# CostaLab/PILOT

Measured on AMD Instinct MI355X. Metric: W2 patient-pairs/sec (full NxN EMD matrix), higher is better.
Workload: dtype f32 (products as 2-way fp16 splits, 22 significant bits, on the f16 MFMA, f32 accumulate)

## Files before the change

### pilot_amd/csrc/generic_kernels.hpp

```cpp
#pragma once
#include <hip/hip_runtime.h>

#include "plan_args.hpp"

namespace pilot {

struct GenericParams {
    const double *P, *M;
    int N, K;
    int n_pairs, row_begin, row_step;
    double reg, tau, stop_thr;
    int max_iter, period;
    double *emd; int *iters; double *err; int *flags;
    double *kws;
    int *queue;
    const int *list;
    const int *list_len;
    int nsplit;
};

#ifndef PILOT_GENERIC_WG
#define PILOT_GENERIC_WG 1024
#endif
constexpr int GENERIC_WG = PILOT_GENERIC_WG, GENERIC_WAVES = GENERIC_WG / 64;

__device__ inline double block_reduce_sum(double x, double *red) {
    for (int off = 32; off >= 1; off >>= 1) x += __shfl_xor(x, off);
    const int wave = threadIdx.x / 64, lane = threadIdx.x % 64;
    __syncthreads();
    if (lane == 0) red[wave] = x;
    __syncthreads();
    double s = 0.0;
    for (int w = 0; w < GENERIC_WG / 64; ++w) s += red[w];
    return s;
}
__device__ inline double wave_tree_sum(double x) {
    for (int off = 32; off >= 1; off >>= 1) x += __shfl_xor(x, off);
    return x;
}
__device__ inline double block_reduce_max(double x, double *red) {
    for (int off = 32; off >= 1; off >>= 1) { const double y = __shfl_xor(x, off); x = y > x ? y : x; }
    const int wave = threadIdx.x / 64, lane = threadIdx.x % 64;
    __syncthreads();
    if (lane == 0) red[wave] = x;
    __syncthreads();
    double s = red[0];
    for (int w = 1; w < GENERIC_WG / 64; ++w) s = red[w] > s ? red[w] : s;
    return s;
}

#ifndef PILOT_PLAN_TU
static __global__ void __launch_bounds__(GENERIC_WG) sinkhorn_generic_kernel(GenericParams p) {
    constexpr bool PLAN = false;
    const PlanArgs *pa = nullptr;
#else
static __global__ void __launch_bounds__(GENERIC_WG) sinkhorn_generic_plan_kernel(GenericParams p, PlanArgs plan_args) {
    constexpr bool PLAN = true;
    const PlanArgs *pa = &plan_args;
#endif
    extern __shared__ double sm[];
    const int K = p.K, N = p.N;
    double *a = sm, *b = a + K, *u = b + K, *v = u + K, *up = v + K, *vp = up + K, *alpha = vp + K, *beta = alpha + K;
    double *red = beta + K;
    double *part = red + GENERIC_WAVES;
    int *qs = reinterpret_cast<int *>(part + p.nsplit * K);
    double *Km = p.kws + (size_t)blockIdx.x * 2 * K * K, *Kt = Km + (size_t)K * K;
    const double reg = p.reg;
    auto build_kernel = [&]() {
        for (int t = threadIdx.x; t < K * K; t += GENERIC_WG) {
            const int i = t / K, j = t % K;
            const double val = exp(-(p.M[t] - alpha[i] - beta[j]) / reg);
            Km[t] = val;
            Kt[(size_t)j * K + i] = val;
        }
        __threadfence_block();
        __syncthreads();
    };
    for (;;) {
        if (threadIdx.x == 0) qs[0] = atomicAdd(p.queue, 1);
        __syncthreads();
        const int item = qs[0];
        __syncthreads();
        if (item >= (PLAN ? pa->n_pairs : (p.list_len ? *p.list_len : p.n_pairs))) break;
        const int q = PLAN ? item : p.list ? p.list[item] : item;
        const int i_s = PLAN ? pa->pair_i[item] : p.row_begin + (q / N) * p.row_step, j_s = PLAN ? pa->pair_j[item] : q % N;
        for (int k = threadIdx.x; k < K; k += GENERIC_WG) {
            a[k] = p.P[(size_t)i_s * K + k]; b[k] = p.P[(size_t)j_s * K + k];
            alpha[k] = 0.0; beta[k] = 0.0; u[k] = 1.0 / K; v[k] = 1.0 / K;
        }
        __syncthreads();
        build_kernel();
        double err = 1.0;
        int iters = 0, nabs = 0, last_abs = -1, flags = 0;
        for (int ii = 0; ii < p.max_iter; ++ii) {
            for (int k = threadIdx.x; k < K; k += GENERIC_WG) { up[k] = u[k]; vp[k] = v[k]; }
            __syncthreads();
            const int wave = threadIdx.x / 64, lane = threadIdx.x % 64;
            const int ns = p.nsplit, sw = wave % ns, og = wave / ns, n_og = GENERIC_WAVES / ns;
            const int c0 = (K * sw) / ns, c1 = (K * (sw + 1)) / ns;
            auto product = [&](const double *X, const double *x, const double *num, double *out) {
                for (int j0 = lane + 256 * og; j0 < K; j0 += 256 * n_og) {
                    double s0 = 0.0, s1 = 0.0, s2 = 0.0, s3 = 0.0;
                    const bool h1 = j0 + 64 < K, h2 = j0 + 128 < K, h3 = j0 + 192 < K;
#pragma unroll 8
                    for (int i = c0; i < c1; ++i) {
                        const double xi = x[i];
                        const double *row = X + (size_t)i * K + j0;
                        s0 += row[0] * xi;
                        if (h1) s1 += row[64] * xi;
                        if (h2) s2 += row[128] * xi;
                        if (h3) s3 += row[192] * xi;
                    }
                    part[sw * K + j0] = s0;
                    if (h1) part[sw * K + j0 + 64] = s1;
                    if (h2) part[sw * K + j0 + 128] = s2;
                    if (h3) part[sw * K + j0 + 192] = s3;
                }
                __syncthreads();
                for (int j = threadIdx.x; j < K; j += GENERIC_WG) {
                    double t = part[j];
                    for (int w = 1; w < ns; ++w) t += part[w * K + j];
                    out[j] = num[j] / t;
                }
                __syncthreads();
            };
            product(Km, u, b, v);
            product(Kt, v, a, u);
            iters = ii + 1;
            double mu = 0.0, mv = 0.0, nanf = 0.0;
            for (int k = threadIdx.x; k < K; k += GENERIC_WG) {
                if (u[k] != u[k] || v[k] != v[k]) nanf = 1.0;
                mu = fabs(u[k]) > mu ? fabs(u[k]) : mu;
                mv = fabs(v[k]) > mv ? fabs(v[k]) : mv;
            }
            const bool has_nan = block_reduce_max(nanf, red) > 0.0;
            mu = block_reduce_max(mu, red);
            mv = block_reduce_max(mv, red);
            if (!has_nan && (mu > p.tau || mv > p.tau)) {
                for (int k = threadIdx.x; k < K; k += GENERIC_WG) {
                    alpha[k] += reg * log(u[k]); u[k] = 1.0 / K;
                    beta[k] += reg * log(v[k]); v[k] = 1.0 / K;
                }
                __syncthreads();
                build_kernel();
                ++nabs; last_abs = ii;
            }
            if (ii % p.period == 0) {
                double e2 = 0.0;
                for (int j = wave; j < K; j += GENERIC_WG / 64) {
                    const double lv = log(v[j]);
                    double s = 0.0;
                    for (int i = lane; i < K; i += 64) s += exp(-(p.M[(size_t)i * K + j] - alpha[i] - beta[j]) / reg + log(u[i]) + lv);
                    s = wave_tree_sum(s);
                    if (lane == 0) e2 += (s - b[j]) * (s - b[j]);
                }
                err = sqrt(block_reduce_sum(e2, red));
            }
            if (err <= p.stop_thr) { flags |= 1; break; }
            if (has_nan) {
                for (int k = threadIdx.x; k < K; k += GENERIC_WG) { u[k] = up[k]; v[k] = vp[k]; }
                __syncthreads();
                flags |= 2;
                break;
            }
        }
        if (last_abs >= 0 && last_abs == iters - 1) flags |= 4;
        if (nabs > 0) flags |= 8;
        double val = 0.0;
        for (int t = threadIdx.x; t < K * K; t += GENERIC_WG) {
            const int i = t / K, j = t % K;
            if constexpr (PLAN) {
                const double g = exp(-(p.M[t] - alpha[i] - beta[j]) / reg + log(u[i]) + log(v[j]));
                pa->plans[(size_t)q * K * K + t] = g;
                val += p.M[t] * g;
            } else {
                val += p.M[t] * exp(-(p.M[t] - alpha[i] - beta[j]) / reg + log(u[i]) + log(v[j]));
            }
        }
        val = block_reduce_sum(val, red);
        if (threadIdx.x == 0) {
            p.emd[q] = val;
            if (p.iters) p.iters[q] = iters;
            if (p.err) p.err[q] = err;
            p.flags[q] = flags | 16;
        }
        __syncthreads();
    }
}

}
```

### pilot_amd/csrc/pilot_ot.hip

```cpp
#include <hip/hip_runtime.h>
#include <pthread.h>

#include <chrono>
#include <cmath>
#include <condition_variable>
#include <cstdarg>
#include <cstdio>
#include <cstdlib>
#include <cstring>
#include <map>
#include <mutex>
#include <string>
#include <thread>
#include <new>
#include <vector>

#include "abi_common.hpp"
#include "sinkhorn_launch.hpp"
#include "emd_kernels.hpp"
#include "emd_multi_kernels.hpp"
#include "prepass_kernels.hpp"
#include "cellw2_kernels.hpp"
#include "generic_kernels.hpp"
#include "emd_generic_kernel.hpp"
// ... 130 lines not shown
            bool neg = false;
            for (int d = 0; d < D; ++d) { neg = neg || u[d] < 0.0 || v[d] < 0.0; su += u[d]; sv += v[d]; }
            if (neg || su == 0.0 || sv == 0.0) { out = HUGE_VAL; break; }
            const double ru = 1.0 / su, rv = 1.0 / sv;
            double js = 0.0;
            for (int d = 0; d < D; ++d) {
                const double p = u[d] * ru, q = v[d] * rv, m = (p + q) / 2.0;
                if (p > 0.0) js += p * log(p / m);
                if (q > 0.0) js += q * log(q / m);
            }
            out = sqrt(js / 2.0);
            break;
        }
        case PILOT_OT_METRIC_MAHALANOBIS: {
            double s = 0.0;
            for (int a = 0; a < D; ++a) {
                double t = 0.0;
                for (int b = 0; b < D; ++b) t += (u[b] - v[b]) * aux[(size_t)b * D + a];
                s += t * (u[a] - v[a]);
            }
            out = sqrt(s);
            break;
        }
        default: {
            double s = 0.0;
            for (int d = 0; d < D; ++d) { const double t = fabs(u[d] - v[d]); s = t > s ? t : s; }
            out = s;
        }
        }
        C[(size_t)i * K + j] = out;
        C[(size_t)j * K + i] = out;
    }
}

constexpr int MAX_K = 128;
constexpr int GENERIC_MAX_K = 2048;
constexpr int EMD_MAX_K = 256;
constexpr int WIDE_MAX_K = 256;
constexpr int CTRL_INTS = pilot::CTRL_INTS;
constexpr int CTRL_SHARDS_AT = (CTRL_INTS + 2 * pilot::ORDER_NB + 31) / 32 * 32;
constexpr int CTRL_SHARDS_TRACK_AT = CTRL_SHARDS_AT + pilot::QUEUE_SHARDS * pilot::QUEUE_SHARD_STRIDE;
constexpr int CTRL_BLOCK_INTS = CTRL_SHARDS_TRACK_AT + pilot::QUEUE_SHARDS * pilot::QUEUE_SHARD_STRIDE;
constexpr int TIMING_RING = 64;

constexpr size_t LDS_BYTES = 160 * 1024;
static int emd_nk(int K) { return K <= 64 ? 1 : (K <= 128 ? 2 : (K <= 192 ? 3 : 4)); }
constexpr int EMD_MULTI_MAX_K = 16;
static int emd_multi_mode(int K) {
    const char *e = pilot::test_switch("PILOT_OT_EMD_MULTI");
    if (e && *e) return atoi(e);
    return K <= 15 ? 1 : 2;
}
static int emd_wgs_per_cu(int K) {
    if (K > 128) return 1;
    const size_t lds = pilot::emd_lds_bytes(K);
    int by_lds = (int)(LDS_BYTES / lds);
    const int by_regs = K <= 64 ? 4 : 2;
    if (by_lds > by_regs) by_lds = by_regs;
    return by_lds < 1 ? 1 : by_lds;
}

}

struct pilot_ot_plan {
    int N, K, device;
    double max_cost;
    void *img;
    void *p_slot;
    int *track_list;
    int *track_count;
    int *order_list;
    unsigned char *order_bucket;
    int *order_hist;
    int *flags_ws;
    size_t flags_ws_n;
    int *emd_counter;
    double *f_slab;
    size_t f_slab_bytes;
    double *emdg_slab;
    int emdg_wgs;
    double *kws;
    int generic_wgs;
    float *wide_rec;
    size_t wide_rec_n;
    int *nan_list;
    size_t nan_list_n;
    int n_cu;
    int timing;
    long n_timed;
    long n_calls;
    hipEvent_t ev[TIMING_RING][4];
    int graph_mode;
    int gkey_seen;
    struct GraphKey {
        const void *P, *M, *emd, *iters, *err, *flags;
        double reg, stop_thr, tau, floor_ulps, max_cost;
        int num_iter_max, check_period, cfg, mixed, sym, row_begin, n_rows, row_step, debug;
        bool operator==(const GraphKey &o) const {
            return P == o.P && M == o.M && emd == o.emd && iters == o.iters && err == o.err && flags == o.flags && reg == o.reg &&
                   stop_thr == o.stop_thr && tau == o.tau && floor_ulps == o.floor_ulps && max_cost == o.max_cost && num_iter_max == o.num_iter_max &&
                   check_period == o.check_period && cfg == o.cfg && mixed == o.mixed && sym == o.sym && row_begin == o.row_begin &&
                   n_rows == o.n_rows && row_step == o.row_step && debug == o.debug;
        }
    } gkey;
    hipStream_t gstream;
    hipGraphExec_t gexec;
};

namespace {
std::mutex g_switch_mutex;
std::map<std::string, std::string> g_switches;
}
namespace pilot {
const char *test_switch(const char *name) {
    static thread_local std::string value;
    std::lock_guard<std::mutex> l(g_switch_mutex);
    if (g_switches.empty()) return nullptr;
    auto it = g_switches.find(name);
    if (it == g_switches.end()) return nullptr;
    value = it->second;
    return value.c_str();
}
}

PILOT_API int pilot_ot_test_switch(const char *name, const char *value) {
    std::lock_guard<std::mutex> l(g_switch_mutex);
    if (!name) { g_switches.clear(); return PILOT_OT_OK; }
    if (value) g_switches[name] = value; else g_switches.erase(name);
    return PILOT_OT_OK;
}

PILOT_API int pilot_ot_version(void) { return PILOT_OT_VERSION; }
PILOT_API const char *pilot_ot_last_error(void) { return g_err; }

PILOT_API int pilot_ot_device_count(int *count) {
    if (!count) return fail(PILOT_OT_EINVAL, "count is NULL");
    int n = 0;
    hipError_t e = hipGetDeviceCount(&n);
    if (e != hipSuccess) { (void)hipGetLastError(); n = 0; }
    *count = n;
    return PILOT_OT_OK;
}

PILOT_API int pilot_ot_get_device(int *device) {
    if (!device) return fail(PILOT_OT_EINVAL, "device is NULL");
    HIP_TRY(hipGetDevice(device));
    return PILOT_OT_OK;
}

PILOT_API int pilot_ot_set_device(int device) {
    HIP_TRY(hipSetDevice(device));
    return PILOT_OT_OK;
}

PILOT_API int pilot_ot_device_name(char *buf, int buflen) {
    if (!buf || buflen <= 0) return fail(PILOT_OT_EINVAL, "bad buffer");
    int dev = 0;
    HIP_TRY(hipGetDevice(&dev));
    hipDeviceProp_t prop;
    HIP_TRY(hipGetDeviceProperties(&prop, dev));
    snprintf(buf, buflen, "%s", prop.gcnArchName);
    return PILOT_OT_OK;
}

PILOT_API int pilot_ot_dev_alloc(void **dptr, unsigned long long bytes) {
    if (!dptr) return fail(PILOT_OT_EINVAL, "dptr is NULL");
    HIP_TRY(hipMalloc(dptr, bytes ? bytes : 1));
    return PILOT_OT_OK;
}
PILOT_API int pilot_ot_dev_free(void *dptr) {
    HIP_TRY(hipFree(dptr));
    return PILOT_OT_OK;
}
PILOT_API int pilot_ot_memcpy_h2d(void *dst, const void *src, unsigned long long bytes) {
    HIP_TRY(hipMemcpy(dst, src, bytes, hipMemcpyHostToDevice));
    return PILOT_OT_OK;
}
PILOT_API int pilot_ot_memcpy_d2h(void *dst, const void *src, unsigned long long bytes) {
    HIP_TRY(hipMemcpy(dst, src, bytes, hipMemcpyDeviceToHost));
    return PILOT_OT_OK;
}
PILOT_API int pilot_ot_stream_sync(void *stream) {
    HIP_TRY(hipStreamSynchronize(static_cast<hipStream_t>(stream)));
    return PILOT_OT_OK;
}

namespace { hipError_t ws_get(int slot, size_t bytes, void **out); }

PILOT_API int pilot_ot_cost_matrix_dev_ex(const double *d_centroids, int K, int D, int metric, const double *d_aux, double *d_cost,
                                          void *stream) {
    if (!d_centroids || !d_cost) return fail(PILOT_OT_EINVAL, "NULL pointer");
    if (K <= 0 || D <= 0) return fail(PILOT_OT_EINVAL, "K=%d D=%d must be positive", K, D);
    if (metric < PILOT_OT_METRIC_COSINE || metric > PILOT_OT_METRIC_MAHALANOBIS)
        return fail(PILOT_OT_EINVAL, "unknown metric id %d", metric);
    if (metric == PILOT_OT_METRIC_MAHALANOBIS && !d_aux) return fail(PILOT_OT_EINVAL, "mahalanobis needs the D x D inverse covariance (aux)");
    if (K > 4096 || D > 4096) return fail(PILOT_OT_ENOTSUP, "K=%d D=%d: at most 4096 centroids / dimensions", K, D);
    hipLaunchKernelGGL(cost_matrix_kernel, dim3(1), dim3(1024), sizeof(double) * (2 * K + D),
                       static_cast<hipStream_t>(stream), d_centroids, K, D, metric, d_aux, d_cost);
    HIP_TRY(hipGetLastError());
    return PILOT_OT_OK;
}

PILOT_API int pilot_ot_cost_matrix_dev(const double *d_centroids, int K, int D, int metric, double *d_cost, void *stream) {
    return pilot_ot_cost_matrix_dev_ex(d_centroids, K, D, metric, nullptr, d_cost, stream);
}

PILOT_API int pilot_ot_cost_matrix_ex(const double *centroids, int K, int D, int metric, const double *aux, double *cost) {
    if (!centroids || !cost) return fail(PILOT_OT_EINVAL, "NULL pointer");
    if (K <= 0 || D <= 0) return fail(PILOT_OT_EINVAL, "K=%d D=%d must be positive", K, D);
    const bool has_aux = metric == PILOT_OT_METRIC_MAHALANOBIS;
    if (has_aux && !aux) return fail(PILOT_OT_EINVAL, "mahalanobis needs the D x D inverse covariance (aux)");
    void *dx = nullptr, *dc = nullptr, *da = nullptr;
    HIP_TRY(ws_get(9, sizeof(double) * (size_t)K * D, &dx));
    HIP_TRY(ws_get(10, sizeof(double) * (size_t)K * K, &dc));
    HIP_TRY(hipMemcpy(dx, centroids, sizeof(double) * (size_t)K * D, hipMemcpyHostToDevice));
    if (has_aux) {
        HIP_TRY(ws_get(11, sizeof(double) * (size_t)D * D, &da));
        HIP_TRY(hipMemcpy(da, aux, sizeof(double) * (size_t)D * D, hipMemcpyHostToDevice));
    }
    const int rc = pilot_ot_cost_matrix_dev_ex(static_cast<double *>(dx), K, D, metric, static_cast<double *>(da), static_cast<double *>(dc), nullptr);
    if (rc != PILOT_OT_OK) return rc;
    HIP_TRY(hipMemcpy(cost, dc, sizeof(double) * (size_t)K * K, hipMemcpyDeviceToHost));
    return PILOT_OT_OK;
}

PILOT_API int pilot_ot_cost_matrix(const double *centroids, int K, int D, int metric, double *cost) {
    return pilot_ot_cost_matrix_ex(centroids, K, D, metric, nullptr, cost);
}

static double h_max_cost_over_reg() {
    const char *e = pilot::test_switch("PILOT_OT_H_MAX_COST_OVER_REG");
    return e && *e ? atof(e) : pilot::H_MAX_COST_OVER_REG;
}

PILOT_API int pilot_ot_auto_precision(double max_cost_over_reg) {
    if (max_cost_over_reg <= h_max_cost_over_reg()) return PILOT_OT_PREC_F16X2;
    return max_cost_over_reg <= 60.0 ? PILOT_OT_PREC_BF16X3 : PILOT_OT_PREC_F64;
}

namespace { bool split_fits_lds(int K, bool sym, int bands); }
PILOT_API int pilot_ot_auto_precision_for(double max_cost_over_reg, int K, int cost_is_symmetric) {
    int prec = pilot_ot_auto_precision(max_cost_over_reg);
    if ((prec == PILOT_OT_PREC_BF16X3 || prec == PILOT_OT_PREC_F16X2) && !split_fits_lds(K, cost_is_symmetric != 0, 1)) prec = PILOT_OT_PREC_F32;
    return prec;
}

PILOT_API int pilot_ot_resolve_precision(int precision, double max_cost_over_reg, int K, int cost_is_symmetric, double tau) {
    if (precision == PILOT_OT_PREC_GENERIC || max_cost_over_reg > PILOT_OT_MAX_COST_OVER_REG) return PILOT_OT_PREC_GENERIC;
    const bool f32_class = precision == PILOT_OT_PREC_F32 || precision == PILOT_OT_PREC_BF16X3 || precision == PILOT_OT_PREC_F16X2;
    const char *raw = pilot::test_switch("PILOT_OT_RAW_PRECISION");
    const bool promote = f32_class && max_cost_over_reg > 60.0 && !(raw && *raw && *raw != '0');
    if (precision == PILOT_OT_PREC_AUTO || promote) {
        precision = pilot_ot_auto_precision_for(max_cost_over_reg, K, cost_is_symmetric);
        if (precision == PILOT_OT_PREC_F64) precision = PILOT_OT_PREC_AUTO_MIXED;
    }
    if (precision == PILOT_OT_PREC_F16X2 &&
        (max_cost_over_reg > h_max_cost_over_reg() || tau > pilot::H_MAX_TAU || !split_fits_lds(K, cost_is_symmetric != 0, 1)))
        precision = split_fits_lds(K, cost_is_symmetric != 0, 1) ? PILOT_OT_PREC_BF16X3 : PILOT_OT_PREC_F32;
    return precision;
}

PILOT_API int pilot_ot_plan_create(int N, int K, pilot_ot_plan **plan) {
    if (!plan) return fail(PILOT_OT_EINVAL, "plan is NULL");
    if (N <= 0 || K <= 0) return fail(PILOT_OT_EINVAL, "N=%d K=%d must be positive", N, K);
    if (K > GENERIC_MAX_K) return fail(PILOT_OT_ENOTSUP, "K=%d > %d cell types", K, GENERIC_MAX_K);
    if ((long long)N * N > 0x7fffffffLL) return fail(PILOT_OT_ENOTSUP, "N=%d: N*N overflows the pair index", N);
    pilot_ot_plan *pl = new (std::nothrow) pilot_ot_plan();
    if (!pl) return fail(PILOT_OT_EINVAL, "out of host memory");
    pl->N = N; pl->K = K; pl->max_cost = 1.0;
    pl->img = nullptr; pl->p_slot = nullptr; pl->track_list = nullptr; pl->track_count = nullptr;
    pl->emd_counter = nullptr; pl->f_slab = nullptr; pl->f_slab_bytes = 0; pl->emdg_slab = nullptr; pl->emdg_wgs = 0; pl->n_cu = 256; pl->kws = nullptr; pl->generic_wgs = 0; pl->nan_list = nullptr; pl->nan_list_n = 0;
    pl->wide_rec = nullptr; pl->wide_rec_n = 0;
    pl->order_list = nullptr; pl->order_bucket = nullptr; pl->order_hist = nullptr;
    pl->flags_ws = nullptr; pl->flags_ws_n = 0;
    pl->timing = 0; pl->n_timed = 0; pl->n_calls = 0;
    pl->graph_mode = 0; pl->gkey_seen = 0; pl->gstream = nullptr; pl->gexec = nullptr;
    for (int i = 0; i < TIMING_RING; ++i) for (int j = 0; j < 4; ++j) pl->ev[i][j] = nullptr;
    hipError_t e = hipGetDevice(&pl->device);
    if (e == hipSuccess) {
        int n_cu = 0;
        if (hipDeviceGetAttribute(&n_cu, hipDeviceAttributeMultiprocessorCount, pl->device) == hipSuccess && n_cu > 0)
            pl->n_cu = n_cu;
    }
    const int kp = ((K + 31) / 32) * 32;
    if (K <= MAX_K) {
        const int rt = (K + 15) / 16;
        size_t img_bytes = pilot::img_elems(pilot::CFG_F64, rt) * sizeof(double);
        const size_t b32 = pilot::img_elems(pilot::CFG_F32, rt) * sizeof(float), bs = pilot::img_elems(pilot::CFG_S32, rt) * sizeof(float);
        const size_t bh = pilot::img_elems(pilot::CFG_H32, rt) * sizeof(float);
        if (b32 > img_bytes) img_bytes = b32;
        if (bs > img_bytes) img_bytes = bs;
        if (bh > img_bytes) img_bytes = bh;
        if (e == hipSuccess) e = hipMalloc(&pl->img, img_bytes);
    } else if (K <= WIDE_MAX_K) {
        if (e == hipSuccess) e = hipMalloc(&pl->img, pilot::img_elems(pilot::CFG_H32, 16) * sizeof(float));
    }
    {
        size_t p_bytes = sizeof(double) * ((size_t)N * kp + N);
        if (K > MAX_K && K <= WIDE_MAX_K) { const size_t two = 2 * sizeof(float) * ((size_t)N * 256 + N); p_bytes = two > p_bytes ? two : p_bytes; }
        if (e == hipSuccess) e = hipMalloc(&pl->p_slot, p_bytes);
    }
    if (e == hipSuccess) e = hipMalloc(reinterpret_cast<void **>(&pl->track_list), sizeof(int) * (size_t)N * N);
    if (e == hipSuccess) e = hipMalloc(reinterpret_cast<void **>(&pl->track_count), CTRL_BLOCK_INTS * sizeof(int));
    if (e == hipSuccess) e = hipMalloc(reinterpret_cast<void **>(&pl->order_list), sizeof(int) * (size_t)N * N);
    if (e == hipSuccess) e = hipMalloc(reinterpret_cast<void **>(&pl->order_bucket), (size_t)N * N);
    if (e == hipSuccess) e = hipMalloc(reinterpret_cast<void **>(&pl->emd_counter), sizeof(int) * pilot::EMD_NQ * pilot::EMD_Q_STRIDE);
    if (e == hipSuccess) e = hipMalloc(reinterpret_cast<void **>(&pl->nan_list), 2 * sizeof(int) * (size_t)N * N);
    if (e == hipSuccess) pl->nan_list_n = (size_t)N * N;
    if (e == hipSuccess) e = hipMalloc(reinterpret_cast<void **>(&pl->flags_ws), sizeof(int) * (size_t)N * N);
    if (e == hipSuccess) pl->flags_ws_n = (size_t)N * N;
    if (e != hipSuccess) {
        pilot_ot_plan_destroy(pl);
        return fail(PILOT_OT_EHIP, "plan allocation failed: %s", hipGetErrorString(e));
    }
    *plan = pl;
    return PILOT_OT_OK;
}

PILOT_API int pilot_ot_plan_set_max_cost(pilot_ot_plan *pl, double max_cost) {
    if (!pl) return fail(PILOT_OT_EINVAL, "plan is NULL");
    if (!(max_cost > 0.0) || !std::isfinite(max_cost)) return fail(PILOT_OT_EINVAL, "max_cost=%g must be positive and finite", max_cost);
    pl->max_cost = max_cost;
    return PILOT_OT_OK;
}

PILOT_API int pilot_ot_plan_destroy(pilot_ot_plan *pl) {
    if (!pl) return PILOT_OT_OK;
    if (pl->img) (void)hipFree(pl->img);
    if (pl->p_slot) (void)hipFree(pl->p_slot);
    if (pl->track_list) (void)hipFree(pl->track_list);
    if (pl->track_count) (void)hipFree(pl->track_count);
    if (pl->order_list) (void)hipFree(pl->order_list);
    if (pl->order_bucket) (void)hipFree(pl->order_bucket);
    if (pl->flags_ws) (void)hipFree(pl->flags_ws);
    if (pl->emd_counter) (void)hipFree(pl->emd_counter);
    if (pl->f_slab) (void)hipFree(pl->f_slab);
    if (pl->emdg_slab) (void)hipFree(pl->emdg_slab);
    if (pl->kws) (void)hipFree(pl->kws);
    if (pl->nan_list) (void)hipFree(pl->nan_list);
    if (pl->wide_rec) (void)hipFree(pl->wide_rec);
    if (pl->gexec) (void)hipGraphExecDestroy(pl->gexec);
    if (pl->gstream) (void)hipStreamDestroy(pl->gstream);
    for (int i = 0; i < TIMING_RING; ++i) for (int j = 0; j < 4; ++j) if (pl->ev[i][j]) (void)hipEventDestroy(pl->ev[i][j]);
    delete pl;
    return PILOT_OT_OK;
}

namespace {

int check_grid_args(int N, int K, double reg, int num_iter_max, double stop_thr, double tau, int check_period,
                    int precision, int row_begin, int row_end, int row_step) {
    if (N <= 0 || K <= 0) return fail(PILOT_OT_EINVAL, "N=%d K=%d must be positive", N, K);
    if (!(reg > 0.0) || !std::isfinite(reg)) return fail(PILOT_OT_EINVAL, "reg=%g must be positive and finite", reg);
    if (num_iter_max < 1) return fail(PILOT_OT_EINVAL, "num_iter_max=%d must be >= 1", num_iter_max);
    if (check_period < 1) return fail(PILOT_OT_EINVAL, "check_period=%d must be >= 1", check_period);
    if (!(stop_thr >= 0.0) || !(stop_thr < 1.0)) return fail(PILOT_OT_EINVAL, "stop_thr=%g must be in [0, 1)", stop_thr);
    if (!(tau > 1.0)) return fail(PILOT_OT_EINVAL, "tau=%g must be > 1", tau);
    if (precision < PILOT_OT_PREC_AUTO || precision > PILOT_OT_PREC_F16X2)
        return fail(PILOT_OT_EINVAL, "unknown precision id %d", precision);
    if (row_step < 1 || row_begin < 0 || row_end > N || row_begin > row_end)
        return fail(PILOT_OT_EINVAL, "bad row range [%d, %d) step %d for N=%d", row_begin, row_end, row_step, N);
    if (K > GENERIC_MAX_K) return fail(PILOT_OT_ENOTSUP, "K=%d > %d cell types", K, GENERIC_MAX_K);
    return PILOT_OT_OK;
}

constexpr double MAX_COST_OVER_REG = PILOT_OT_MAX_COST_OVER_REG;

int run_generic(pilot_ot_plan *pl, const double *d_P, const double *d_M, double reg, int num_iter_max, double stop_thr, double tau,
                int check_period, int row_begin, int n_rows, int row_step, double *d_emd, int *d_iters, double *d_err, int *d_flags,
                hipStream_t s, const int *list = nullptr, const int *list_len = nullptr, int *queue = nullptr) {
    const int N = pl->N, K = pl->K;
    const int n_pairs = n_rows * N;
    if (n_pairs == 0) return PILOT_OT_OK;
    int nsplit = pilot::GENERIC_WAVES;
    auto lds_for = [&](int ns) { return sizeof(double) * ((8 + (size_t)ns) * (size_t)K + pilot::GENERIC_WAVES) + 16; };
    while (nsplit > 1 && lds_for(nsplit) > LDS_BYTES) nsplit /= 2;
    const size_t lds = lds_for(nsplit);
    if (lds > LDS_BYTES) return fail(PILOT_OT_ENOTSUP, "K=%d does not fit the generic kernel's LDS vectors", K);
    if (!pl->kws) {
        int wgs = 3 * pl->n_cu;
        const size_t per = sizeof(double) * 2 * (size_t)K * K;
        while (wgs > 1 && per * wgs > ((size_t)8 << 30)) wgs /= 2;
        HIP_TRY(hipMalloc(reinterpret_cast<void **>(&pl->kws), per * wgs));
        pl->generic_wgs = wgs;
    }
    if (!d_flags) {
        if ((size_t)n_pairs > pl->flags_ws_n) {
            if (pl->flags_ws) HIP_TRY(hipFree(pl->flags_ws));
            pl->flags_ws = nullptr; pl->flags_ws_n = 0;
            HIP_TRY(hipMalloc(reinterpret_cast<void **>(&pl->flags_ws), sizeof(int) * (size_t)n_pairs));
            pl->flags_ws_n = (size_t)n_pairs;
        }
        d_flags = pl->flags_ws;
    }
    if (!queue) { queue = pl->track_count; HIP_TRY(hipMemsetAsync(queue, 0, sizeof(int), s)); }
    pilot::GenericParams g;
    g.P = d_P; g.M = d_M; g.N = N; g.K = K; g.n_pairs = n_pairs; g.row_begin = row_begin; g.row_step = row_step;
    g.reg = reg; g.tau = tau; g.stop_thr = stop_thr; g.max_iter = num_iter_max; g.period = check_period;
    g.emd = d_emd; g.iters = d_iters; g.err = d_err; g.flags = d_flags; g.kws = pl->kws; g.queue = queue; g.nsplit = nsplit;
    g.list = list; g.list_len = list_len;
    int wgs = pl->generic_wgs < n_pairs ? pl->generic_wgs : n_pairs;
    if (list && wgs > 64) wgs = 64;
    if (const char *e = pilot::test_switch("PILOT_OT_GENERIC_WGS")) { const int w = atoi(e); if (w > 0 && w < wgs) wgs = w; }
    HIP_TRY(hipFuncSetAttribute(reinterpret_cast<const void *>(pilot::sinkhorn_generic_kernel), hipFuncAttributeMaxDynamicSharedMemorySize, (int)lds));
    hipLaunchKernelGGL(pilot::sinkhorn_generic_kernel, dim3(wgs), dim3(pilot::GENERIC_WG), lds, s, g);
    HIP_TRY(hipGetLastError());
    return PILOT_OT_OK;
}

int stream_min_waves(int w , int RT, bool sym, bool track, int tv, bool split, bool half = false) {
    if (half && !track && RT <= pilot::HALF_OCC4_MAX_RT) return 4;
    if (split) return RT <= (track ? pilot::SPLIT_OCC2_MAX_RT_TRACK : (half ? pilot::HALF_OCC2_MAX_RT : pilot::SPLIT_OCC2_MAX_RT)) ? 2 : 1;
    const int na = RT * 4 * RT * w;
    const bool greg = !split && sym && na <= pilot::GREG_MAX;
    const int regs = (track ? 7 : 5) * RT * 4 * w + 4 * w + 56 + (tv ? 24 * w : 0) + (split ? 3 * ((RT + 1) / 2) * 4 + 24 : 0) +
                     (greg ? na + 2 * tv * ((RT - 1) * 4 + 1) * w : 0);
    return regs <= 128 ? 4 : (regs <= 168 ? 3 : (regs <= 256 ? 2 : 1));
}
bool stream_has_solo(int w, int RT, bool sym, int tv, bool split, bool half) {
    const int mw = stream_min_waves(w, RT, sym, false, tv, split, half);
    const int budget = mw >= 4 ? 128 : (mw == 3 ? 168 : 256);
    return sym && RT <= 4 && !(half && RT < pilot::HALF_SOLO_MIN_RT) && (64 + 45) * w <= budget;
}

struct StreamLds { size_t bytes; int ring, wgs_per_cu; };
StreamLds stream_lds(size_t fixed, size_t slot_bytes, int want, int min_ring = 4) {
    StreamLds r;
    for (;;) {
        const size_t budget = LDS_BYTES / (size_t)want;
        long ring = budget > fixed ? (long)((budget - fixed) / ((size_t)pilot::WAVES_PER_WG * slot_bytes)) : 0;
        if (ring >= min_ring || want == 1) {
            if (ring > pilot::RING_MAX) ring = pilot::RING_MAX;
            if (ring < 1) ring = 0;
            r.ring = (int)ring; r.wgs_per_cu = want;
            r.bytes = fixed + (size_t)pilot::WAVES_PER_WG * slot_bytes * (size_t)ring;
            return r;
        }
        --want;
    }
}

bool split_fits_lds(int K, bool sym, int bands = 1) {
    const int RT = (K + 15) / 16, KP = RT * 16;
    const size_t fixed = (size_t)(sym ? 1 : 2) * pilot::form_elems_rt(pilot::CFG_S32, RT) * 4 * bands + (size_t)KP * 4 +
                         (size_t)pilot::WAVES_PER_WG * pilot::HANDOVER_BUF * sizeof(int);
    return fixed + (size_t)4 * pilot::WAVES_PER_WG * (2 * KP + 4) * 4 <= LDS_BYTES;
}

int run_grid(int cfg, pilot_ot_plan *pl, const double *d_P, const double *d_M, double reg, int num_iter_max,
             double stop_thr, double tau, int check_period, double floor_ulps, bool sym, int row_begin,
             int n_rows, int row_step, double *d_emd, int *d_iters, double *d_err, int *d_flags, hipStream_t s,
             bool mixed = false) {
    const bool f64 = cfg == pilot::CFG_F64, half = cfg == pilot::CFG_H32, split = cfg == pilot::CFG_S32 || half;
    const size_t ts = f64 ? sizeof(double) : sizeof(float);
    const int w = (int)(ts / 4);
    constexpr int TILE = 16;
    const int N = pl->N, K = pl->K;
    const int RT = (K + TILE - 1) / TILE;
    const int KP = RT * TILE;
    const char *dbg = pilot::test_switch("PILOT_OT_DEBUG");
    const int debug = dbg ? atoi(dbg) : 0;
    const size_t form = pilot::form_elems_rt(cfg, RT);
    const size_t hb_bytes = (size_t)pilot::WAVES_PER_WG * pilot::HANDOVER_BUF * sizeof(int);
    size_t fixed = (size_t)(sym ? 1 : 2) * form * ts + (size_t)KP * ts + hb_bytes;
    int tv = 0;
    const int live1 = (split && RT >= 2 && RT <= 4 && K - (RT - 1) * TILE <= 4) ? 1 : 0;
    if (!split) {
        const int n_tail = K - (RT - 1) * TILE;
        if (RT >= 2 && RT <= 7 && n_tail <= 4 && !(debug & 256)) tv = n_tail <= 2 ? 1 : 2;
        const size_t tail_lds = (size_t)(sym ? 1 : 2) * tv * ((RT - 1) * 4 + 1) * 64 * 2 * ts;
        if (tv && fixed + tail_lds + 4 * pilot::WAVES_PER_WG * (2 * KP + 4) * ts > LDS_BYTES) tv = 0;
        if (tv) fixed += tail_lds;
    }
    const size_t slot_bytes = (size_t)(2 * KP + 4) * ts;
    if (fixed + pilot::WAVES_PER_WG * slot_bytes > LDS_BYTES)
        return fail(PILOT_OT_ENOTSUP, "K=%d with a %ssymmetric cost needs %zu B of LDS (> %zu) in this precision", K, sym ? "" : "non-",
                    fixed + pilot::WAVES_PER_WG * slot_bytes, LDS_BYTES);
    pl->order_hist = pl->track_count + CTRL_INTS;
    HIP_TRY(hipMemsetAsync(pl->track_count, 0, CTRL_BLOCK_INTS * sizeof(int), s));
    void *img = pl->img;
    void *Pt = pl->p_slot;
    if (n_rows == 0) return PILOT_OT_OK;

    const int n_pairs = n_rows * N;
    if (!d_flags) {
        if ((size_t)n_pairs > pl->flags_ws_n) {
            if (pl->flags_ws) HIP_TRY(hipFree(pl->flags_ws));
            pl->flags_ws = nullptr; pl->flags_ws_n = 0;
            HIP_TRY(hipMalloc(reinterpret_cast<void **>(&pl->flags_ws), sizeof(int) * (size_t)n_pairs));
            pl->flags_ws_n = (size_t)n_pairs;
        }
        d_flags = pl->flags_ws;
    }

    pilot::GridParams p;
    p.P = Pt; p.img = img; p.N = N; p.K = K;
    p.n_pairs = n_pairs;
    p.list = nullptr; p.list_len = nullptr;
    p.solo_len = nullptr; p.solo_head = nullptr; p.solo_blocks = 0;
    p.row_begin = row_begin; p.row_step = row_step;
    p.max_iter = num_iter_max; p.period = check_period;
    p.stop_thr = stop_thr; p.tau = tau; p.floor_ulps = floor_ulps;
    p.emd = d_emd; p.iters = d_iters; p.err = d_err; p.flags = d_flags;
    p.track_list = pl->track_list; p.track_count = pl->track_count; p.queue_head = pl->track_count + 1;
    p.queue_shards = pl->track_count + CTRL_SHARDS_AT;
    p.ring = 0;
    p.fb_list = nullptr; p.fb_count = nullptr; p.bands = 1;
    if ((size_t)n_pairs > pl->nan_list_n) {
        if (pl->nan_list) HIP_TRY(hipFree(pl->nan_list));
        pl->nan_list = nullptr; pl->nan_list_n = 0;
        HIP_TRY(hipMalloc(reinterpret_cast<void **>(&pl->nan_list), 2 * sizeof(int) * (size_t)n_pairs));
        pl->nan_list_n = (size_t)n_pairs;
    }
    p.nan_list = pl->nan_list; p.nan_count = pl->track_count + 10;
    p.unequal = pl->track_count + pilot::CTRL_UNEQUAL;
    const bool redo64 = !mixed && split && pl->max_cost / reg > 12.0 && !(debug & 4096);
    const bool track_all = mixed || (split && !half && pl->max_cost / reg > 24.0 && !(debug & 8192));
    int *const fb_list = pl->nan_list + pl->nan_list_n;
    if (redo64) { p.fb_list = fb_list; p.fb_count = pl->track_count + 8; }
    p.debug = debug;
    const int tiles = (n_pairs + TILE - 1) / TILE;
    const long full_tiles = ((long)N * N + TILE - 1) / TILE;
    const long wave_slots = (long)pl->n_cu * stream_min_waves(w, RT, sym, false, tv, split, half) * pilot::WAVES_PER_WG;
    const bool solo = stream_has_solo(w, RT, sym, tv, split, half) && !(p.debug & 512) && !track_all && full_tiles < 3 * wave_slots;
    int solo_blocks = 0;
    {
        int ob = (n_pairs + 1023) / 1024;
        if (ob > pl->n_cu) ob = pl->n_cu;
        int *split_ctl = pl->track_count + 4;
        const int mode = (solo ? 2 : 0) | ((p.debug & 2) ? 4 : 0);
        HIP_TRY(pilot::launch_prep(cfg, d_M, K, RT, reg, img, d_P, Pt, N, (tv ? 1 : 0) | 2 | (mixed ? 4 : 0), stop_thr, floor_ulps, n_rows, row_begin, row_step,
                                   pl->order_bucket, pl->order_hist, pl->order_list, split_ctl, pl->track_count + 1, mode, ob, s));
        p.list = pl->order_list;
        if (solo) {
            solo_blocks = (n_rows + pilot::WAVES_PER_WG - 1) / pilot::WAVES_PER_WG;
            if (solo_blocks > pl->n_cu) solo_blocks = pl->n_cu;
            p.solo_len = split_ctl + 3; p.solo_head = pl->track_count + 3; p.solo_blocks = solo_blocks;
        }
    }
    hipEvent_t *ev = (pl->timing > 0 && (pl->n_calls++ % pl->timing) == 0) ? pl->ev[pl->n_timed % TIMING_RING] : nullptr;
    if (ev) HIP_TRY(hipEventRecord(ev[0], s));
    const bool quad = half && pilot::quad_covers(K, sym) && !pilot::test_switch("PILOT_OT_NO_QUAD");
    auto launch = [&](int tvv, bool track, int wgs, const StreamLds &L) -> hipError_t {
        p.ring = L.ring;
        if (tvv) return pilot::launch_stream_tv(cfg, tvv, RT, sym, track, dim3(wgs), L.bytes, s, p);
        if (half && !track && quad) return pilot::launch_quad(dim3(wgs), s, p);
        if (half && !track) return pilot::launch_stream_h32(RT, sym, live1, dim3(wgs), L.bytes, s, p);
        if (split) return pilot::launch_stream_s32(RT, sym, track, live1, dim3(wgs), L.bytes, s, p);
        return f64 ? pilot::launch_stream_f64(RT, sym, track, dim3(wgs), L.bytes, s, p)
                   : pilot::launch_stream_f32(RT, sym, track, dim3(wgs), L.bytes, s, p);
    };
    if (!track_all && quad) {
        int wgs = 2 * pl->n_cu;
        if (wgs > tiles) wgs = tiles;
        HIP_TRY(launch(tv, false, wgs, StreamLds{}));
    } else if (!track_all) {
        int want = stream_min_waves(w, RT, sym, false, tv, split, half);
        if (half && K <= 4 && want > 2) want = 2;
        if ((p.debug >> 4) & 7) want = (p.debug >> 4) & 7;
        const bool park = split && RT <= 4;
        const size_t slot_fast = half ? (size_t)pilot::ring_slot_stride<pilot::CfgH32x16>(RT) * ts : slot_bytes;
        const size_t park_lane = half ? (size_t)pilot::park_lane_elems<pilot::CfgH32x16>(RT) : (size_t)RT * 4;
        const size_t park_bytes = park ? (size_t)pilot::WAVES_PER_WG * park_lane * 64 * ts : 0;
        if (fixed + park_bytes + pilot::WAVES_PER_WG * slot_fast > LDS_BYTES)
            return fail(PILOT_OT_ENOTSUP, "K=%d: operand images + ring + park area exceed LDS", K);
        const StreamLds L = stream_lds(fixed + park_bytes, slot_fast, want);
        int wgs = pl->n_cu * L.wgs_per_cu;
        const int need = (tiles + pilot::WAVES_PER_WG - 1) / pilot::WAVES_PER_WG;
        if (wgs > need) wgs = need;
        wgs += solo_blocks;
        HIP_TRY(launch(tv, false, wgs, L));
    }
    if (ev) { HIP_TRY(hipEventRecord(ev[1], s)); HIP_TRY(hipEventRecord(ev[2], s)); }
    p.list = pl->track_list; p.list_len = pl->track_count; p.queue_head = pl->track_count + 2;
    p.queue_shards = pl->track_count + CTRL_SHARDS_TRACK_AT;
    p.solo_blocks = 0;
    size_t fixed_t = fixed;
    if (half) {
        p.img = static_cast<float *>(img) + pilot::track_img_elems(cfg, RT);
        fixed_t = (size_t)(sym ? 1 : 2) * pilot::form_elems_rt(pilot::CFG_S32, RT) * ts + (size_t)KP * ts + hb_bytes;
    }
    if (track_all) { p.list = pl->order_list; p.list_len = nullptr; }
    if (mixed) {
        p.bands = 2;
        p.fb_list = pl->track_list; p.fb_count = pl->track_count + 8;
        fixed_t = (size_t)(sym ? 1 : 2) * form * ts * 2 + (size_t)KP * ts + hb_bytes;
    }
    {
        const int tv_t = RT <= 4 ? tv : 0;
        const StreamLds L = stream_lds(fixed_t, slot_bytes, stream_min_waves(w, RT, sym, true, tv_t, split));
        int wgs_t = pl->n_cu * L.wgs_per_cu;
        const int need = (tiles + pilot::WAVES_PER_WG - 1) / pilot::WAVES_PER_WG;
        if (wgs_t > need) wgs_t = need;
        HIP_TRY(launch(tv_t, true, wgs_t, L));
    }
    if (mixed || redo64) {
        const int RT64 = RT;
        const size_t form64 = pilot::form_elems_rt(pilot::CFG_F64, RT64);
        const size_t fixed64 = (size_t)(sym ? 1 : 2) * form64 * sizeof(double) + (size_t)KP * sizeof(double);
        const size_t slot64 = (size_t)(2 * KP + 4) * sizeof(double);
        if (fixed64 + pilot::WAVES_PER_WG * slot64 > LDS_BYTES)
            return fail(PILOT_OT_ENOTSUP, "K=%d: the f64 fallback needs %zu B of LDS", K, fixed64 + pilot::WAVES_PER_WG * slot64);
        HIP_TRY(pilot::launch_prep(pilot::CFG_F64, d_M, K, RT64, reg, img, d_P, Pt, N, 2, stop_thr, floor_ulps, 0, row_begin, row_step,
                                   pl->order_bucket, pl->order_hist, pl->order_list, pl->track_count + 4, pl->track_count + 1, 0, 1, s));
        pilot::GridParams q = p;
        q.list = mixed ? pl->track_list : fb_list; q.list_len = pl->track_count + 8; q.queue_head = pl->track_count + 9; q.queue_shards = nullptr;
        q.img = img;
        q.fb_list = nullptr; q.fb_count = nullptr; q.bands = 1;
        q.nan_list = pl->nan_list; q.nan_count = pl->track_count + 10;
        if (sym && K <= 64 && !(p.debug & 2048)) {
            HIP_TRY(pilot::launch_solo_track_f64(dim3(64), s, q));
        } else {
            const StreamLds L = stream_lds(fixed64, slot64, stream_min_waves(2, RT64, sym, true, 0, false));
            q.ring = L.ring;
            int wgs_t = pl->n_cu * L.wgs_per_cu;
            const int need = (tiles + pilot::WAVES_PER_WG - 1) / pilot::WAVES_PER_WG;
            if (wgs_t > need) wgs_t = need;
            HIP_TRY(pilot::launch_stream_f64(RT64, sym, true, dim3(wgs_t), L.bytes, s, q));
        }
    }
    if (ev) { HIP_TRY(hipEventRecord(ev[3], s)); ++pl->n_timed; }
    if (!(p.debug & 1024)) {
        const int rc = run_generic(pl, d_P, d_M, reg, num_iter_max, stop_thr, tau, check_period, row_begin, n_rows, row_step, d_emd, d_iters,
                                   d_err, d_flags, s, pl->nan_list, pl->track_count + 10, pl->track_count + 11);
        if (rc != PILOT_OT_OK) return rc;
    }
    return PILOT_OT_OK;
}

int run_wide(pilot_ot_plan *pl, const double *d_P, const double *d_M, double reg, int num_iter_max, double stop_thr, double tau,
             int check_period, double floor_ulps, int row_begin, int n_rows, int row_step, double *d_emd, int *d_iters, double *d_err,
             int *d_flags, hipStream_t s) {
    const int N = pl->N, K = pl->K, RT = 16;
    long WIDE_CHUNK_PAIRS = 512L * 1024;
    if (const char *e = pilot::test_switch("PILOT_OT_WIDE_CHUNK")) { const long v = atol(e); if (v > 0) WIDE_CHUNK_PAIRS = v; }
    if ((long)n_rows * N > WIDE_CHUNK_PAIRS && n_rows > 1) {
        const int rows_per = (int)(WIDE_CHUNK_PAIRS / N) > 0 ? (int)(WIDE_CHUNK_PAIRS / N) : 1;
        for (int r0 = 0; r0 < n_rows; r0 += rows_per) {
            const int nr = n_rows - r0 < rows_per ? n_rows - r0 : rows_per;
            const size_t off = (size_t)r0 * N;
            const int rc = run_wide(pl, d_P, d_M, reg, num_iter_max, stop_thr, tau, check_period, floor_ulps, row_begin + r0 * row_step, nr, row_step,
                                    d_emd + off, d_iters ? d_iters + off : nullptr, d_err ? d_err + off : nullptr, d_flags ? d_flags + off : nullptr, s);
            if (rc != PILOT_OT_OK) return rc;
        }
        return PILOT_OT_OK;
    }
    pl->order_hist = pl->track_count + CTRL_INTS;
    HIP_TRY(hipMemsetAsync(pl->track_count, 0, (CTRL_INTS + 2 * pilot::ORDER_NB) * sizeof(int), s));
    if (n_rows == 0) return PILOT_OT_OK;
    const int n_pairs = n_rows * N;
    if (!d_flags) {
        if ((size_t)n_pairs > pl->flags_ws_n) {
            if (pl->flags_ws) HIP_TRY(hipFree(pl->flags_ws));
            pl->flags_ws = nullptr; pl->flags_ws_n = 0;
            HIP_TRY(hipMalloc(reinterpret_cast<void **>(&pl->flags_ws), sizeof(int) * (size_t)n_pairs));
            pl->flags_ws_n = (size_t)n_pairs;
        }
        d_flags = pl->flags_ws;
    }
    if ((size_t)n_pairs > pl->nan_list_n) {
        if (pl->nan_list) HIP_TRY(hipFree(pl->nan_list));
        pl->nan_list = nullptr; pl->nan_list_n = 0;
        HIP_TRY(hipMalloc(reinterpret_cast<void **>(&pl->nan_list), 2 * sizeof(int) * (size_t)n_pairs));
        pl->nan_list_n = (size_t)n_pairs;
    }
    if ((size_t)n_pairs > pl->wide_rec_n) {
        if (pl->wide_rec) HIP_TRY(hipFree(pl->wide_rec));
        pl->wide_rec = nullptr; pl->wide_rec_n = 0;
        HIP_TRY(hipMalloc(reinterpret_cast<void **>(&pl->wide_rec), sizeof(float) * pilot::wide_rec_elems() * (size_t)n_pairs));
        pl->wide_rec_n = (size_t)n_pairs;
    }
    int ob = (n_pairs + 1023) / 1024;
    if (ob > pl->n_cu) ob = pl->n_cu;
    HIP_TRY(pilot::launch_prep(pilot::CFG_H32, d_M, K, RT, reg, pl->img, d_P, pl->p_slot, N, 0, stop_thr, floor_ulps, n_rows, row_begin, row_step,
                               pl->order_bucket, pl->order_hist, pl->order_list, pl->track_count + 4, pl->track_count + 1, 0, ob, s));
    pilot::GridParams p;
    p.P = pl->p_slot; p.img = pl->img; p.N = N; p.K = K;
    p.n_pairs = n_pairs;
    p.list = pl->order_list; p.list_len = nullptr;
    p.solo_len = nullptr; p.solo_head = nullptr; p.solo_blocks = 0;
    p.row_begin = row_begin; p.row_step = row_step;
    p.max_iter = num_iter_max; p.period = check_period;
    p.stop_thr = stop_thr; p.tau = tau; p.floor_ulps = floor_ulps;
    p.emd = d_emd; p.iters = d_iters; p.err = d_err; p.flags = d_flags;
    p.track_list = pl->track_list; p.track_count = pl->track_count; p.queue_head = pl->track_count + 1; p.queue_shards = nullptr;
    p.ring = 0; p.bands = 1;
    p.fb_list = nullptr; p.fb_count = nullptr;
    p.nan_list = pl->nan_list; p.nan_count = pl->track_count + 10;
    p.unequal = pl->track_count + pilot::CTRL_UNEQUAL;
    p.debug = 0;
    hipEvent_t *ev = (pl->timing > 0 && (pl->n_calls++ % pl->timing) == 0) ? pl->ev[pl->n_timed % TIMING_RING] : nullptr;
    if (ev) HIP_TRY(hipEventRecord(ev[0], s));
    const int tiles = (n_pairs + 15) / 16;
    int wgs = pl->n_cu < tiles ? pl->n_cu : tiles;
    HIP_TRY(pilot::launch_wide(dim3(wgs), s, p, pl->wide_rec));
    if (ev) { HIP_TRY(hipEventRecord(ev[1], s)); HIP_TRY(hipEventRecord(ev[2], s)); }
    int vwgs = (tiles + pilot::WAVES_PER_WG - 1) / pilot::WAVES_PER_WG;
    if (vwgs > 2 * pl->n_cu) vwgs = 2 * pl->n_cu;
    HIP_TRY(pilot::launch_wide_value(dim3(vwgs), s, p, pl->wide_rec));
    if (ev) { HIP_TRY(hipEventRecord(ev[3], s)); ++pl->n_timed; }
    return run_generic(pl, d_P, d_M, reg, num_iter_max, stop_thr, tau, check_period, row_begin, n_rows, row_step, d_emd, d_iters, d_err,
                       d_flags, s, pl->nan_list, pl->track_count + 10, pl->track_count + 11);
}

}

PILOT_API int pilot_ot_sinkhorn_grid_dev(pilot_ot_plan *pl, const double *d_P, const double *d_M, double reg,
                                         int num_iter_max, double stop_thr, double tau, int check_period,
                                         int precision, double f32_floor_ulps, int cost_is_symmetric,
                                         int row_begin, int row_end, int row_step, double *d_emd, int *d_iters,
                                         double *d_err, int *d_flags, void *stream) {
    if (!pl || !d_P || !d_M || !d_emd) return fail(PILOT_OT_EINVAL, "NULL pointer");
    int rc = check_grid_args(pl->N, pl->K, reg, num_iter_max, stop_thr, tau, check_period, precision, row_begin,
                             row_end, row_step);
    if (rc != PILOT_OT_OK) return rc;
    {
        const int n_rows_g = (row_end - row_begin + row_step - 1) / row_step;
        if (pl->K > MAX_K && pl->K <= WIDE_MAX_K && cost_is_symmetric && precision != PILOT_OT_PREC_GENERIC && precision != PILOT_OT_PREC_F64 &&
            pl->max_cost / reg <= h_max_cost_over_reg() && tau <= pilot::H_MAX_TAU && !pilot::test_switch("PILOT_OT_NO_WIDE")) {
            if (!(f32_floor_ulps > 0.0)) f32_floor_ulps = 8.0;
            return run_wide(pl, d_P, d_M, reg, num_iter_max, stop_thr, tau, check_period, f32_floor_ulps, row_begin, n_rows_g, row_step, d_emd,
                            d_iters, d_err, d_flags, static_cast<hipStream_t>(stream));
        }
        if (precision == PILOT_OT_PREC_GENERIC || pl->K > MAX_K || pl->max_cost / reg > MAX_COST_OVER_REG)
            return run_generic(pl, d_P, d_M, reg, num_iter_max, stop_thr, tau, check_period, row_begin, n_rows_g, row_step, d_emd,
                               d_iters, d_err, d_flags, static_cast<hipStream_t>(stream));
    }
    precision = pilot_ot_resolve_precision(precision, pl->max_cost / reg, pl->K, cost_is_symmetric, tau);
    bool mixed = false;
    if (precision == PILOT_OT_PREC_AUTO_MIXED) {
        precision = PILOT_OT_PREC_F64;
        mixed = true;
    }
    mixed = mixed && split_fits_lds(pl->K, cost_is_symmetric != 0, 2) && pl->max_cost / reg <= 140.0 && !pilot::test_switch("PILOT_OT_NO_MIXED");
    if (!(f32_floor_ulps > 0.0)) f32_floor_ulps = 8.0;
    const int n_rows = (row_end - row_begin + row_step - 1) / row_step;
    hipStream_t s = static_cast<hipStream_t>(stream);
    const int cfg = mixed ? pilot::CFG_S32
                          : (precision == PILOT_OT_PREC_F32 ? pilot::CFG_F32
                             : (precision == PILOT_OT_PREC_BF16X3 ? pilot::CFG_S32 : (precision == PILOT_OT_PREC_F16X2 ? pilot::CFG_H32 : pilot::CFG_F64)));
    auto run = [&](hipStream_t on) {
        int r = run_grid(cfg, pl, d_P, d_M, reg, num_iter_max, stop_thr, tau, check_period, f32_floor_ulps, cost_is_symmetric != 0,
                         row_begin, n_rows, row_step, d_emd, d_iters, d_err, d_flags, on, mixed);
        if (r == PILOT_OT_ENOTSUP)
            r = run_generic(pl, d_P, d_M, reg, num_iter_max, stop_thr, tau, check_period, row_begin, n_rows, row_step, d_emd, d_iters, d_err,
                            d_flags, on);
        return r;
    };
    if (!pl->graph_mode || pl->timing || n_rows == 0) return run(s);
    const char *dbg = pilot::test_switch("PILOT_OT_DEBUG");
    const pilot_ot_plan::GraphKey key = {d_P, d_M, d_emd, d_iters, d_err, d_flags, reg, stop_thr, tau, f32_floor_ulps, pl->max_cost, num_iter_max,
                                         check_period, cfg, mixed ? 1 : 0, cost_is_symmetric != 0 ? 1 : 0, row_begin, n_rows, row_step,
                                         dbg ? atoi(dbg) : 0};
    if (pl->gexec && key == pl->gkey) {
        HIP_TRY(hipGraphLaunch(pl->gexec, s));
        return PILOT_OT_OK;
    }
    if (pl->gexec) { (void)hipGraphExecDestroy(pl->gexec); pl->gexec = nullptr; }
    if (!(pl->gkey_seen && key == pl->gkey)) {
        pl->gkey = key; pl->gkey_seen = 1;
        return run(s);
    }
    if (!pl->gstream) HIP_TRY(hipStreamCreateWithFlags(&pl->gstream, hipStreamNonBlocking));
    HIP_TRY(hipStreamBeginCapture(pl->gstream, hipStreamCaptureModeThreadLocal));
    rc = run(pl->gstream);
    hipGraph_t graph = nullptr;
    const hipError_t ce = hipStreamEndCapture(pl->gstream, &graph);
    if (rc != PILOT_OT_OK) { if (graph) (void)hipGraphDestroy(graph); return rc; }
    if (ce != hipSuccess) { (void)hipGetLastError(); return fail(PILOT_OT_EHIP, "graph capture failed: %s", hipGetErrorString(ce)); }
    const hipError_t ie = hipGraphInstantiate(&pl->gexec, graph, nullptr, nullptr, 0);
    (void)hipGraphDestroy(graph);
    if (ie != hipSuccess) { (void)hipGetLastError(); pl->gexec = nullptr; return fail(PILOT_OT_EHIP, "graph instantiation failed: %s", hipGetErrorString(ie)); }
    HIP_TRY(hipGraphLaunch(pl->gexec, s));
    return PILOT_OT_OK;
}

PILOT_API int pilot_ot_plan_enable_graph(pilot_ot_plan *pl, int enable) {
    if (!pl) return fail(PILOT_OT_EINVAL, "plan is NULL");
    pl->graph_mode = enable ? 1 : 0;
    if (!enable) {
        if (pl->gexec) { (void)hipGraphExecDestroy(pl->gexec); pl->gexec = nullptr; }
        pl->gkey_seen = 0;
    }
    return PILOT_OT_OK;
}

namespace {
struct WsPool {
    static constexpr int SLOTS = 48;
    void *p[SLOTS] = {};
    size_t cap[SLOTS] = {};
    int device = -1;
    void release() {
        for (int i = 0; i < SLOTS; ++i) { if (p[i]) (void)hipFree(p[i]); p[i] = nullptr; cap[i] = 0; }
        device = -1;
    }
    hipError_t get(int slot, size_t bytes, void **out) {
        int dev = 0;
        hipError_t e = hipGetDevice(&dev);
        if (e != hipSuccess) return e;
        if (dev != device) { release(); device = dev; }
        if (bytes > cap[slot]) {
            if (p[slot]) (void)hipFree(p[slot]);
            p[slot] = nullptr; cap[slot] = 0;
            const size_t want = bytes + bytes / 4 + 256;
            e = hipMalloc(&p[slot], want);
            if (e != hipSuccess) return e;
            cap[slot] = want;
        }
        *out = p[slot];
        return hipSuccess;
    }
};
struct HostCtx {
    pilot_ot_plan *plan = nullptr;
    int N = 0, K = 0, device = -1;
    size_t n_out = 0;
    double *dP = nullptr, *dM = nullptr, *dE = nullptr, *dErr = nullptr;
    int *dIt = nullptr, *dFl = nullptr;
    unsigned char *pin = nullptr;
    size_t pin_bytes = 0;
    static constexpr int FETCH_EVENTS = 32;
    hipEvent_t fev[FETCH_EVENTS];
    int n_fev = 0;
    void release() {
        for (int i = 0; i < n_fev; ++i) (void)hipEventDestroy(fev[i]);
        n_fev = 0;
        if (pin) (void)hipHostFree(pin);
        pin = nullptr; pin_bytes = 0;
        if (dP) (void)hipFree(dP);
        if (dM) (void)hipFree(dM);
        if (dE) (void)hipFree(dE);
        if (dErr) (void)hipFree(dErr);
        if (dIt) (void)hipFree(dIt);
        if (dFl) (void)hipFree(dFl);
        dP = dM = dE = dErr = nullptr; dIt = dFl = nullptr;
        if (plan) pilot_ot_plan_destroy(plan);
        plan = nullptr; N = K = 0; n_out = 0; device = -1;
    }
    ~HostCtx() {}
};
struct PrepassClock {
    hipEvent_t ev[2] = {nullptr, nullptr};
    bool valid = false;
    void release() { for (auto &e : ev) { if (e) (void)hipEventDestroy(e); e = nullptr; } valid = false; }
    void start() {
        valid = false;
        if (!ev[0] && (hipEventCreate(&ev[0]) != hipSuccess || hipEventCreate(&ev[1]) != hipSuccess)) { release(); return; }
        (void)hipEventRecord(ev[0], nullptr);
    }
    void stop() { if (ev[1]) valid = hipEventRecord(ev[1], nullptr) == hipSuccess; }
};
struct ThreadCtx { HostCtx host; WsPool ws; PrepassClock clock; bool orphan = false; };
std::mutex g_tctx_mutex;
std::vector<ThreadCtx *> g_tctx_all;
struct TctxOwner {
    ThreadCtx *c = nullptr;
    ~TctxOwner() {
        if (!c) return;
        std::lock_guard<std::mutex> l(g_tctx_mutex);
        c->orphan = true;
    }
};
thread_local TctxOwner g_tctx_owner;
ThreadCtx &tctx() {
    if (!g_tctx_owner.c) {
        std::lock_guard<std::mutex> l(g_tctx_mutex);
        for (size_t i = 0; i < g_tctx_all.size();) {
            if (g_tctx_all[i]->orphan) {
                g_tctx_all[i]->host.release();
                g_tctx_all[i]->ws.release();
                g_tctx_all[i]->clock.release();
                delete g_tctx_all[i];
                g_tctx_all.erase(g_tctx_all.begin() + (long)i);
            } else {
                ++i;
            }
        }
        g_tctx_owner.c = new ThreadCtx();
        g_tctx_all.push_back(g_tctx_owner.c);
    }
    return *g_tctx_owner.c;
}
#define g_host (tctx().host)
#define g_ws (tctx().ws)
#define g_clock (tctx().clock)
hipError_t ws_get(int slot, size_t bytes, void **out) { return g_ws.get(slot, bytes, out); }
}
namespace pilot {
hipError_t ws_buffer(int slot, size_t bytes, void **out) { return ws_get(slot, bytes, out); }
}
namespace {

int host_ctx_prepare(int N, int K, size_t n_out) {
    int dev = 0;
    HIP_TRY(hipGetDevice(&dev));
    HostCtx &h = g_host;
    if (h.plan && (h.N != N || h.K != K || h.device != dev)) h.release();
    if (!h.plan) {
        int rc = pilot_ot_plan_create(N, K, &h.plan);
        if (rc != PILOT_OT_OK) return rc;
        h.N = N; h.K = K; h.device = dev;
        hipError_t e = hipMalloc(&h.dP, sizeof(double) * (size_t)N * K);
        if (e == hipSuccess) e = hipMalloc(&h.dM, sizeof(double) * (size_t)K * K);
        if (e != hipSuccess) { h.release(); return fail(PILOT_OT_EHIP, "device staging failed: %s", hipGetErrorString(e)); }
    }
    if (n_out > h.n_out) {
        if (h.dE) (void)hipFree(h.dE);
        if (h.dErr) (void)hipFree(h.dErr);
        if (h.dIt) (void)hipFree(h.dIt);
        if (h.dFl) (void)hipFree(h.dFl);
        h.dE = h.dErr = nullptr; h.dIt = h.dFl = nullptr; h.n_out = 0;
        hipError_t e = hipMalloc(&h.dE, sizeof(double) * n_out);
        if (e == hipSuccess) e = hipMalloc(&h.dErr, sizeof(double) * n_out);
        if (e == hipSuccess) e = hipMalloc(reinterpret_cast<void **>(&h.dIt), sizeof(int) * n_out);
        if (e == hipSuccess) e = hipMalloc(reinterpret_cast<void **>(&h.dFl), sizeof(int) * n_out);
        if (e != hipSuccess) { h.release(); return fail(PILOT_OT_EHIP, "device staging failed: %s", hipGetErrorString(e)); }
        h.n_out = n_out;
    }
    const size_t need = n_out * (2 * sizeof(double) + 2 * sizeof(int)) + 4 * 64;
    if (need > h.pin_bytes) {
        if (h.pin) (void)hipHostFree(h.pin);
        h.pin = nullptr; h.pin_bytes = 0;
        if (hipHostMalloc(reinterpret_cast<void **>(&h.pin), need, hipHostMallocDefault) != hipSuccess) {
            (void)hipGetLastError();
            h.pin = nullptr;
        } else {
            h.pin_bytes = need;
        }
    }
    return PILOT_OT_OK;
}

struct CopyJob { void *dst; const void *src; size_t bytes; int *left; };
class CopyPool {
public:
    static constexpr int HELPERS = 2;
    static CopyPool *get() {
        static std::once_flag once;
        std::call_once(once, [] {
            g_pool = new (std::nothrow) CopyPool();
            pthread_atfork(nullptr, nullptr, [] { g_pool = nullptr; });
        });
        return g_pool;
    }
    void push(void *dst, const void *src, size_t bytes, int *left) {
        { std::lock_guard<std::mutex> l(m_); ++*left; q_.push_back(CopyJob{dst, src, bytes, left}); }
        cv_.notify_one();
    }
    void finish(int *left) {
        std::unique_lock<std::mutex> l(m_);
        while (*left > 0) {
            if (!q_.empty()) run_one(l);
            else done_.wait(l);
        }
    }
    int helpers() const { return n_started_; }
private:
    CopyPool() {
        for (int t = 0; t < HELPERS; ++t) {
            try { std::thread([this] { loop(); }).detach(); ++n_started_; }
            catch (...) { break; }
        }
    }
    void run_one(std::unique_lock<std::mutex> &l) {
        const CopyJob j = q_.back(); q_.pop_back();
        l.unlock();
        memcpy(j.dst, j.src, j.bytes);
        l.lock();
        if (--*j.left == 0) done_.notify_all();
    }
    void loop() {
        std::unique_lock<std::mutex> l(m_);
        for (;;) {
            cv_.wait(l, [this] { return !q_.empty(); });
            run_one(l);
        }
    }
    static CopyPool *g_pool;
    std::mutex m_;
    std::condition_variable cv_, done_;
    std::vector<CopyJob> q_;
    int n_started_ = 0;
};
CopyPool *CopyPool::g_pool = nullptr;

struct Fetch { void *dst; const void *src; size_t bytes; };
int host_fetch(const Fetch *f, int n) {
    HostCtx &h = g_host;
    if (!h.pin) {
        HIP_TRY(hipStreamSynchronize(nullptr));
        for (int i = 0; i < n; ++i)
            if (f[i].dst) HIP_TRY(hipMemcpy(f[i].dst, f[i].src, f[i].bytes, hipMemcpyDeviceToHost));
        return PILOT_OT_OK;
    }
    size_t total = 0;
    for (int i = 0; i < n; ++i) if (f[i].dst) total += f[i].bytes;
    constexpr size_t PIPELINE_FROM = (size_t)1 << 20;
    int want_threads = 1 + CopyPool::HELPERS;
    if (const char *e = pilot::test_switch("PILOT_OT_FETCH_THREADS")) { const int w = atoi(e); if (w >= 1 && w < want_threads) want_threads = w; }
    CopyPool *pool = (total >= PIPELINE_FROM && want_threads > 1) ? CopyPool::get() : nullptr;
    if (!pool || pool->helpers() == 0) {
        size_t off = 0;
        for (int i = 0; i < n; ++i) {
            if (!f[i].dst) continue;
            HIP_TRY(hipMemcpyAsync(h.pin + off, f[i].src, f[i].bytes, hipMemcpyDeviceToHost, nullptr));
            off += (f[i].bytes + 63) & ~(size_t)63;
        }
        HIP_TRY(hipStreamSynchronize(nullptr));
        off = 0;
        for (int i = 0; i < n; ++i) {
            if (!f[i].dst) continue;
            memcpy(f[i].dst, h.pin + off, f[i].bytes);
            off += (f[i].bytes + 63) & ~(size_t)63;
        }
        return PILOT_OT_OK;
    }
    while (h.n_fev < HostCtx::FETCH_EVENTS) {
        HIP_TRY(hipEventCreateWithFlags(&h.fev[h.n_fev], hipEventDisableTiming));
        ++h.n_fev;
    }
    struct Piece { unsigned char *dst; const unsigned char *pin; size_t bytes; };
    Piece pieces[HostCtx::FETCH_EVENTS];
    int n_pieces = 0;
    size_t piece = (size_t)768 << 10;
    while ((total + piece - 1) / piece + (size_t)n > (size_t)HostCtx::FETCH_EVENTS) piece *= 2;
    size_t off = 0;
    for (int i = 0; i < n; ++i) {
        if (!f[i].dst) continue;
        for (size_t o = 0; o < f[i].bytes; o += piece) {
            const size_t b = f[i].bytes - o < piece ? f[i].bytes - o : piece;
            HIP_TRY(hipMemcpyAsync(h.pin + off + o, static_cast<const unsigned char *>(f[i].src) + o, b, hipMemcpyDeviceToHost, nullptr));
            HIP_TRY(hipEventRecord(h.fev[n_pieces], nullptr));
            pieces[n_pieces++] = Piece{static_cast<unsigned char *>(f[i].dst) + o, h.pin + off + o, b};
        }
        off += (f[i].bytes + 63) & ~(size_t)63;
    }
    hipError_t err = hipSuccess;
    int left = 0;
    for (int i = 0; i < n_pieces && err == hipSuccess; ++i) {
        err = hipEventSynchronize(h.fev[i]);
        if (err != hipSuccess) break;
        const size_t part = ((pieces[i].bytes + want_threads - 1) / want_threads + 4095) & ~(size_t)4095;
        for (size_t o = 0; o < pieces[i].bytes; o += part)
            pool->push(pieces[i].dst + o, pieces[i].pin + o, pieces[i].bytes - o < part ? pieces[i].bytes - o : part, &left);
    }
// ... 757 lines not shown
```

### pilot_amd/csrc/sinkhorn_kernels.hpp

```cpp
#pragma once
#include <hip/hip_runtime.h>

namespace pilot {

constexpr int WAVE = 64;
constexpr int WAVES_PER_WG = 4;

constexpr int FLAG_CONVERGED = 1, FLAG_NAN = 2, FLAG_ABSORB_LAST = 4, FLAG_ABSORBED = 8, FLAG_F64 = 16;


struct CfgF32x32 {
    using T = float;
    static constexpr bool SPLIT = false, HALF = false;
    static constexpr int NP = 0;
    static constexpr int TILE = 32, NREG = 16, NGRP = 2, VEC = 4;
    using acc_t = float __attribute__((ext_vector_type(16)));
    using vec4_t = float __attribute__((ext_vector_type(4)));
    __host__ __device__ static constexpr int lidx(int t, int r, int g) { return 2 * (16 * t + r) + g; }
    __host__ __device__ static constexpr int lidx_of_row(int t, int p) {
        return lidx(t, (p & 3) + 4 * (p >> 3), (p >> 2) & 1);
    }
    __device__ static inline acc_t mfma(float a, float b, acc_t c) {
        return __builtin_amdgcn_mfma_f32_32x32x2f32(a, b, c, 0, 0, 0);
    }
// ... 1251 lines not shown
#pragma unroll
                    for (int r = 0; r < NREG; ++r) X[t][r] = dead(t, r) ? T(0) : A[t][r] * M::rcp(ACC[t][r]);
                quot_panel(X, PU);
            }
            {
                unsigned int pend = 0u;
                bool have = false;
#pragma unroll
                for (int kb = 0; kb < KB; ++kb)
#pragma unroll
                    for (int h = 0; h < 4; ++h)
                        if (pieces_live(kb, h)) {
                            if (have) { m2 = pk_max3_f16(m2, pend, PU.p[0][kb][h]); have = false; }
                            else { pend = PU.p[0][kb][h]; have = true; }
                        }
                if (have) m2 = pk_max3_f16(m2, pend, pend);
            }
            const f16x2_t mh = __builtin_bit_cast(f16x2_t, m2);
            const float m0 = float(mh[0]), m1 = float(mh[1]);
            mx = (m0 <= tau && m1 <= tau) ? fmax(m0, m1) : __builtin_inff();
        } else {
#pragma unroll
        for (int t = 0; t < RT; ++t)
#pragma unroll
            for (int r = 0; r < NREG; ++r) {
                if (dead(t, r)) continue;
                V[t][r] = B[t][r] * M::rcp(ACC[t][r]);
            }
        product(a_g, w_g, V, ACC, PADC);
#pragma unroll
        for (int t = 0; t < RT; ++t)
#pragma unroll
            for (int r = 0; r < NREG; ++r) {
                if (dead(t, r)) continue;
                const T un = A[t][r] * M::rcp(ACC[t][r]);
                U[t][r] = un;
                if constexpr (TRACK) mx = fmax(fmax(mx, un * RU[t][r]), V[t][r] * RV[t][r]);
                else mx = fmax(fmax(mx, un), V[t][r]);
            }
        }
        const unsigned long long omask = column_any_mask<C>(active && mx > tau);
        const bool over = (omask >> col) & 1ull;
        if constexpr (TRACK) {
            if (over) {
#pragma unroll
                for (int t = 0; t < RT; ++t)
#pragma unroll
                    for (int r = 0; r < NREG; ++r) {
                        const bool pad = M::lidx(t, r, grp) >= K;
                        RU[t][r] = pad ? T(0) : M::rcp(U[t][r] * T(K));
                        RV[t][r] = pad ? T(0) : T(K) * M::rcp(V[t][r]);
                    }
                abs_at = ii;
                flags |= FLAG_ABSORBED;
            }
            if (omask) {
                constexpr T BIG = sizeof(T) == 4 ? T(1.2676506e30) : T(8.452712498170644e270);
                constexpr T SMALL = T(1) / BIG;
                bool z = false;
#pragma unroll
                for (int t = 0; t < RT; ++t)
#pragma unroll
                    for (int r = 0; r < NREG; ++r)
                        z = z || (M::lidx(t, r, grp) < K && !(U[t][r] >= SMALL && U[t][r] < BIG && V[t][r] >= SMALL && V[t][r] < BIG));
                const unsigned long long zmask = column_any_mask<C>(over && z);
                if ((zmask >> col) & 1ull) U[0][0] = __builtin_nanf("");
            }
        }
        auto hand_over = [&]() {
            if (omask) {
                if (over) {
                    if (grp == 0) hb[hb_cnt + (int)__popcll(omask & ((1ull << col) - 1ull))] = q;
                    active = false;
                    want = true;
                }
                hb_cnt += (int)__popcll(omask);
                if (hb_cnt >= HANDOVER_FLUSH) hb_flush();
            }
        };
        if constexpr (!TRACK && !(C::HALF && PILOT_DEFER_HANDOVER)) hand_over();
        ++ii;

        if constexpr (C::HALF) product_h(a_gt.img, PU, ACC);
        else product(a_gt, w_gt, U, ACC, PADC);
        if constexpr (!TRACK && C::HALF && PILOT_DEFER_HANDOVER) hand_over();

        const bool pending = active && ii == chk;
        if (pending) chk += p.period;
        const bool capped = active && ii >= p.max_iter;
        auto lane_e2 = [&](T sc) {
            T e2 = T(0);
            if constexpr (PILOT_E2_PACKED && sizeof(T) == 4 && !TRACK && NREG == 4) {
                using P2 = pair_of<float>;
                P2 acc2 = {0.f, 0.f};
#pragma unroll
                for (int t = 0; t < RT; ++t)
#pragma unroll
                    for (int h = 0; h < 2; ++h) {
                        const int r0 = 2 * h, r1 = 2 * h + 1;
                        if (dead(t, r0) && dead(t, r1)) continue;
                        if (dead(t, r0) || dead(t, r1)) {
                            const int r = dead(t, r0) ? r1 : r0;
                            const float d = V[t][r] * ACC[t][r] - B[t][r];
                            acc2[0] = __builtin_fmaf(d, d, acc2[0]);
                            continue;
                        }
                        const P2 v2 = {V[t][r0], V[t][r1]}, a2 = {ACC[t][r0], ACC[t][r1]}, b2 = {B[t][r0], B[t][r1]};
                        const P2 d2 = __builtin_elementwise_fma(v2, a2, -b2);
                        acc2 = __builtin_elementwise_fma(d2, d2, acc2);
                    }
                return acc2[0] + acc2[1];
            }
#pragma unroll
            for (int t = 0; t < RT; ++t) {
                T et = T(0);
#pragma unroll
                for (int r = 0; r < NREG; ++r) {
                    if (dead(t, r)) continue;
                    T d;
                    if constexpr (TRACK) d = V[t][r] * ACC[t][r] * sc - B[t][r];
                    else d = V[t][r] * ACC[t][r] - B[t][r];
                    et += d * d;
                }
                e2 += et;
            }
            return e2;
        };
        constexpr bool E2_EARLY = C::SPLIT && !TRACK && PILOT_E2_EARLY;
        T e2_early = T(0);
        if constexpr (E2_EARLY) e2_early = lane_e2(T(1));
        if (ballot_b(pending || capped)) {
            T sc = T(1);
            if constexpr (TRACK) sc = (abs_at == ii - 1) ? T(1) / kk : T(1);
            T e2 = E2_EARLY ? e2_early : lane_e2(sc);
            e2 = group_sum<C>(e2);
            const T e = sqrt(e2);
            bool fin = capped;
            if (pending) {
                errv = e;
                if (e <= thr) { fin = true; flags |= FLAG_CONVERGED; }
                else if (e != e) { fin = true; flags |= FLAG_NAN; }
            }
            unsigned long long fmask = ballot_b(fin) & colmask;
            if (fmask) {
                T scale = T(1);
                if constexpr (TRACK) {
                    if (fin && abs_at >= 0 && abs_at == ii - 1) { scale = T(1) / kk; flags |= FLAG_ABSORB_LAST; }
                }
                if constexpr (sizeof(T) == 8) flags |= FLAG_F64;
                if (fin && grp == 0) {
                    if (p.iters) p.iters[q] = ii;
                    if (p.err) p.err[q] = double(errv) * double(T(1) / IN_SCALE);
                }
                while (fmask) {
                    if constexpr (PARK) {
                        if (ring_cnt > 0 && ring_cnt + (int)__popcll(fmask) > p.ring) {
                            if constexpr (C::HALF) {
#pragma unroll
                                for (int part = 0; part < 2; ++part)
#pragma unroll
                                    for (int kb = 0; kb < KB; ++kb) *reinterpret_cast<u32x4_t *>(park + (part * KB + kb) * 4 * WAVE) = PU.p[part][kb];
                            } else {
#pragma unroll
                            for (int t = 0; t < RT; ++t) store_regs<C>(park + t * NREG * WAVE, U[t]);
                            }
                            ring_flush_body<C, RT>(ring, p, ring_cnt);
                            ring_cnt = 0;
                            __builtin_amdgcn_fence(__ATOMIC_ACQUIRE, "workgroup");
                            const int i = p.row_begin + (q / N) * p.row_step, j = q % N;
                            const T *pa = Pt + (size_t)i * KP + grp * NREG, *pb = Pt + (size_t)j * KP + grp * NREG;
                            if constexpr (C::HALF) {
#pragma unroll
                                for (int part = 0; part < 2; ++part)
#pragma unroll
                                    for (int kb = 0; kb < KB; ++kb) PU.p[part][kb] = *reinterpret_cast<const u32x4_t *>(park + (part * KB + kb) * 4 * WAVE);
                            }
#pragma unroll
                            for (int t = 0; t < RT; ++t) {
                                if constexpr (!C::HALF) load_regs<C>(park + t * NREG * WAVE, U[t]);
#pragma unroll
                                for (int r = 0; r < NREG; ++r) { A[t][r] = T(0); B[t][r] = T(0); }
                                if (active) {
                                    load_regs<C>(pa + t * NGRP * NREG, A[t]);
                                    load_regs<C>(pb + t * NGRP * NREG, B[t]);
                                }
                            }
                            if constexpr (C::HALF) product_h(a_gt.img, PU, ACC);
                            else product(a_gt, w_gt, U, ACC, PADC);
                        }
                    }
                    const int space = p.ring - ring_cnt;
                    const int rank = (int)__popcll(fmask & ((1ull << col) - 1ull));
                    const bool put = fin && ((fmask >> col) & 1ull) && rank < space;
                    if (put) {
                        T *rec = ring + (ring_cnt + rank) * RSTRIDE;
                        constexpr int PE = ring_panel_elems<C>(RT);
                        if constexpr (C::HALF) {
#pragma unroll
                            for (int part = 0; part < 2; ++part)
#pragma unroll
                                for (int kb = 0; kb < KB; ++kb)
                                    *reinterpret_cast<u32x4_t *>(rec + ((part * KB + kb) * NGRP + grp) * 4) = PU.p[part][kb];
                            static_assert(!C::HALF || PE >= RT * C::TILE, "the v half of a ring slot holds f32 values");
#pragma unroll
                            for (int t = 0; t < RT; ++t) store_regs<C>(rec + PE + (t * NGRP + grp) * NREG, V[t]);
                        } else {
#pragma unroll
                        for (int t = 0; t < RT; ++t) {
                            store_regs<C>(rec + (t * NGRP + grp) * NREG, U[t]);
                            store_regs<C>(rec + KP + (t * NGRP + grp) * NREG, V[t]);
                        }
                        }
                        if (grp == 0) {
                            rec[2 * PE] = scale;
                            int *meta = reinterpret_cast<int *>(rec + 2 * PE + 1);
                            meta[0] = q;
                            meta[1] = flags;
                        }
                    }
                    const unsigned long long taken = ballot_b(put) & colmask;
                    fmask &= ~taken;
                    ring_cnt = __builtin_amdgcn_readfirstlane(ring_cnt + (int)__popcll(taken));
                    if constexpr (!PARK) {
                        if (ring_cnt >= p.ring) { flush(ring_cnt); ring_cnt = 0; }
                    }
                }
                if (fin) { active = false; want = true; }
            }
        }
    }
    if (ring_cnt > 0) {
        if constexpr (PARK) ring_flush_body<C, RT>(ring, p, ring_cnt);
        else flush(ring_cnt);
    }
    if constexpr (!TRACK) {
        if (hb_cnt > 0) hb_flush();
    }
}

__device__ inline unsigned short bf16_bits(float x) {
    return __builtin_bit_cast(unsigned short, static_cast<__bf16>(x));
}
__device__ inline unsigned short f16_bits(float x) {
    return __builtin_bit_cast(unsigned short, static_cast<_Float16>(x));
}
template <class C>
__device__ inline void write_split_forms(const double *__restrict__ Msrc, int K, int RT, double reg, float *__restrict__ img,
                                         bool two_bands, int tid, int nthr) {
    using M = C;
    const int nimg = form_elems<C>(RT);
    const int KB = split_kblocks(RT);
    unsigned short *im16 = reinterpret_cast<unsigned short *>(img);
    for (int idx = tid; idx < KB * RT * WAVE * 8; idx += nthr) {
        const int e = idx % 8;
        int rest = idx / 8;
        const int lane = rest % WAVE; rest /= WAVE;
        const int t = rest % RT;
        const int kb = rest / RT;
        const int orow = M::lidx_of_row(t, lane % M::TILE);
        const int kt = 2 * kb + e / 4;
        const int k = kt < RT ? M::lidx(kt, e % 4, lane / M::TILE) : K;
        float f[3] = {0.f, 0.f, 0.f}, f1[3] = {0.f, 0.f, 0.f};
        if (orow < K && k < K) {
            const double m_ko = Msrc[(size_t)k * K + orow], m_ok = Msrc[(size_t)orow * K + k];
            const double sc = C::HALF ? double(H_GIBBS_SCALE) : 1.0;
            f[0] = float(exp(-m_ko / reg) * sc);
            f[1] = float(exp(-m_ok / reg) * sc);
            f[2] = float(exp(-m_ok / reg) * m_ok * sc);
            if (two_bands) {
                if (f[0] < SPLIT_SAFE_MIN) { f1[0] = float(exp(-m_ko / reg + BAND1_UP_LN)); f[0] = 0.f; }
                if (f[1] < SPLIT_SAFE_MIN) {
                    f1[1] = float(exp(-m_ok / reg + BAND1_UP_LN));
                    f1[2] = float(exp(-m_ok / reg + BAND1_UP_LN) * m_ok);
                    f[1] = 0.f; f[2] = 0.f;
                }
            }
        }
        if (two_bands) {
            unsigned short *im1 = reinterpret_cast<unsigned short *>(img + band1_offset<C>(RT));
#pragma unroll
            for (int form = 0; form < 3; ++form) {
                float x = f1[form];
#pragma unroll
                for (int part = 0; part < C::NP; ++part) {
                    const unsigned short hb = bf16_bits(x);
                    im1[(size_t)form * nimg * 2 + ((((size_t)part * KB + kb) * RT + t) * WAVE + lane) * 8 + e] = hb;
                    x -= __uint_as_float((unsigned int)hb << 16);
                }
            }
        }
#pragma unroll
        for (int form = 0; form < 3; ++form) {
            float x = f[form];
#pragma unroll
            for (int part = 0; part < C::NP; ++part) {
                unsigned short hb;
                if constexpr (C::HALF) { hb = f16_bits(x); x -= float(__builtin_bit_cast(_Float16, hb)); }
                else { hb = bf16_bits(x); x -= __uint_as_float((unsigned int)hb << 16); }
                im16[(size_t)form * nimg * 2 + ((((size_t)part * KB + kb) * RT + t) * WAVE + lane) * 8 + e] = hb;
            }
        }
    }
}
template <class C>
__device__ inline void write_first_product(const double *__restrict__ Msrc, int K, int RT, double reg, typename C::T *__restrict__ tab,
                                           double scale, int tid, int nthr) {
    using M = C;
    using T = typename C::T;
    const int KP = RT * M::TILE;
    for (int idx = tid; idx < 4 * KP; idx += nthr) {
        const int part = idx & 3, slot = idx >> 2;
        const int r = slot % M::NREG;
        const int g = (slot / M::NREG) % M::NGRP;
        const int t = slot / (M::NGRP * M::NREG);
        const int j = M::lidx(t, r, g);
        double s = 0.0;
        if (j < K)
            for (int k = part; k < K; k += 4) s += exp(-Msrc[(size_t)k * K + j] / reg);
        s += __shfl_xor(s, 1);
        s += __shfl_xor(s, 2);
        if (part == 0) tab[slot] = T(j < K ? s / K * scale : 1.0);
    }
}

template <class C>
__device__ inline void setup_body(const double *__restrict__ Msrc, int K, int RT, double reg,
                                  typename C::T *__restrict__ img, const double *__restrict__ Psrc,
                                  typename C::T *__restrict__ Pdst, long n_p, int write_tail, double stop_thr,
                                  double floor_ulps, int tid, int nthr, int *unequal = nullptr) {
    using M = C;
    using T = typename C::T;
    const int KP = RT * M::TILE;
    const int nimg = form_elems<C>(RT);
    if constexpr (C::SPLIT) {
        write_split_forms<C>(Msrc, K, RT, reg, img, (write_tail & 4) != 0, tid, nthr);
        if constexpr (C::HALF) {
            write_split_forms<CfgS32x16>(Msrc, K, RT, reg, img + track_img_offset<C>(RT), false, tid, nthr);
            write_first_product<CfgS32x16>(Msrc, K, RT, reg, img + track_img_offset<C>(RT) + acc0_offset<CfgS32x16>(RT), 1.0, tid, nthr);
        }
    } else {
    for (int idx = tid; idx < nimg; idx += nthr) {
        const int lane = idx % WAVE;
        int rest = idx / WAVE;
        const int t = rest % RT; rest /= RT;
        const int r = rest % M::NREG;
        const int tp = rest / M::NREG;
        const int orow = M::lidx_of_row(t, lane % M::TILE);
        const int k = M::lidx(tp, r, lane / M::TILE);
        double gt = 0.0, g = 0.0, gm = 0.0;
        if (orow < K && k < K) {
            const double m_ko = Msrc[(size_t)k * K + orow], m_ok = Msrc[(size_t)orow * K + k];
            gt = exp(-m_ko / reg);
            g = exp(-m_ok / reg);
            gm = g * m_ok;
        }
        img[idx] = T(gt);
        img[nimg + idx] = T(g);
        img[2 * nimg + idx] = T(gm);
    }
    }
    write_first_product<C>(Msrc, K, RT, reg, img + acc0_offset<C>(RT), C::HALF ? double(H_GIBBS_SCALE) * double(H_PANEL_SCALE) : 1.0, tid, nthr);
    if (write_tail & 2) {
        T *plain = img + plain_offset<C>(RT);
        for (int idx = tid; idx < 3 * 64 * WAVE; idx += nthr) {
            const int lane = idx % WAVE, k = (idx / WAVE) % 64, tbl = idx / (64 * WAVE);
            double v = 0.0;
            if (k < K && lane < K) {
                if (tbl == 1) v = exp(-Msrc[(size_t)k * K + lane] / reg);
                else v = exp(-Msrc[(size_t)lane * K + k] / reg);
                if (tbl == 2) v *= Msrc[(size_t)lane * K + k];
            }
            plain[idx] = T(v);
        }
    }
    if (write_tail & 1) {
        const int nst = (RT - 1) * 4 + 1;
        T *tail = img + tail_offset<C>(RT);
        for (int idx = tid; idx < 2 * 2 * nst * WAVE * 2; idx += nthr) {
            const int h = idx & 1;
            int rest = idx >> 1;
            const int lane = rest % WAVE; rest /= WAVE;
            const int st = rest % nst; rest /= nst;
            const int c = rest & 1, form = rest >> 1;
            const int row = M::lidx(RT - 1, 0, 2 * c + h);
            const int k = M::lidx(st / M::NREG, st % M::NREG, lane / M::TILE);
            double v = 0.0;
            if (row < K && k < K) v = form == 0 ? exp(-Msrc[(size_t)k * K + row] / reg) : exp(-Msrc[(size_t)row * K + k] / reg);
            tail[idx] = T(v);
        }
    }
    double mass0 = 0.0;
    for (int k = 0; k < K; ++k) mass0 += Psrc[k];
    for (long row = tid; row < n_p / KP; row += nthr) {
        double n2 = 0.0, mass = 0.0;
        for (int k = 0; k < K; ++k) { n2 += Psrc[row * K + k] * Psrc[row * K + k]; mass += Psrc[row * K + k]; }
        if (unequal && !(fabs(mass - mass0) <= 1e-6 * fabs(mass0))) atomicOr(unequal, 1);
        double thr = stop_thr;
        if (sizeof(T) == 4) { const double fl = floor_ulps * 1.1920928955078125e-07 * sqrt(n2); thr = thr > fl ? thr : fl; }
        Pdst[n_p + row] = T(thr);
        if constexpr (C::HALF) Pdst[(n_p + n_p / KP) + n_p + row] = T(thr) * T(H_IN_SCALE);
    }
    for (long idx = tid; idx < n_p; idx += nthr) {
        const long row = idx / KP;
        const int sidx = (int)(idx % KP);
        const int r = sidx % M::NREG, g = (sidx / M::NREG) % M::NGRP, t = sidx / (M::NGRP * M::NREG);
        const int l = M::lidx(t, r, g);
        Pdst[idx] = l < K ? T(Psrc[row * K + l]) : T(0);
        if constexpr (C::HALF) Pdst[(n_p + n_p / KP) + idx] = l < K ? T(Psrc[row * K + l]) * T(H_IN_SCALE) : T(0);
    }
}

constexpr int ORDER_NB = 48;
constexpr int CTRL_INTS = 16, CTRL_UNEQUAL = 12;

__device__ inline int lds_count_aggregated(int *counters, int b, bool valid) {
    int slot = 0;
    unsigned long long todo = ballot_b(valid);
    while (todo) {
        const int leader = __builtin_ctzll(todo);
        const int b0 = __builtin_amdgcn_readlane(b, leader);
        const unsigned long long same = ballot_b(valid && b == b0);
        const int lane = threadIdx.x % WAVE;
        int base = 0;
        if (lane == leader) base = atomicAdd(&counters[b0], (int)__popcll(same));
        base = __builtin_amdgcn_readlane(base, leader);
        if (valid && b == b0) slot = base + (int)__popcll(same & ((1ull << lane) - 1ull));
        todo &= ~same;
    }
    return slot;
}

constexpr int ORDER_JW = 128, ORDER_RI = 8;

__device__ inline void bucket_body(int tile, const double *__restrict__ Psrc, int N, int K, int n_rows, int row_begin,
                                   int row_step, unsigned char *__restrict__ bucket, int *__restrict__ hist, int collapse,
                                   unsigned char *order_smem) {
    const int K4 = (K + 3) & ~3;
    float *Bt = reinterpret_cast<float *>(order_smem);
    float *Ar = Bt + (size_t)K4 * (ORDER_JW + 1);
    int *lh = reinterpret_cast<int *>(Ar + ORDER_RI * K4);
    const int n_jb = (N + ORDER_JW - 1) / ORDER_JW;
    const int jb = (tile % n_jb) * ORDER_JW, rb = (tile / n_jb) * ORDER_RI;
    const int nj = N - jb < ORDER_JW ? N - jb : ORDER_JW;
    const int nr = n_rows - rb < ORDER_RI ? n_rows - rb : ORDER_RI;
    for (int e = threadIdx.x; e < ORDER_NB; e += blockDim.x) lh[e] = 0;
    for (int e = threadIdx.x; e < nj * K; e += blockDim.x) {
        const int row = e / K, k = e % K;
        Bt[k * (ORDER_JW + 1) + row] = float(Psrc[(size_t)jb * K + e]);
    }
    for (int e = threadIdx.x; e < (K4 - K) * ORDER_JW; e += blockDim.x) Bt[(K + e / ORDER_JW) * (ORDER_JW + 1) + e % ORDER_JW] = 0.f;
    for (int e = threadIdx.x; e < ORDER_RI * K4; e += blockDim.x) {
        const int r = e / K4, k = e % K4;
        Ar[e] = (r < nr && k < K) ? float(Psrc[(size_t)(row_begin + (rb + r) * row_step) * K + k]) : 0.f;
    }
    __syncthreads();
    constexpr int R = ORDER_RI / 2;
    const int jl = threadIdx.x % ORDER_JW, half = threadIdx.x / ORDER_JW;
    float l1[R];
#pragma unroll
    for (int r = 0; r < R; ++r) l1[r] = 0.f;
    using f4 = float __attribute__((ext_vector_type(4)));
    for (int k = 0; k < K4; k += 4) {
        float bv[4];
#pragma unroll
        for (int e = 0; e < 4; ++e) bv[e] = Bt[(k + e) * (ORDER_JW + 1) + jl];
#pragma unroll
        for (int r = 0; r < R; ++r) {
            const f4 av = *reinterpret_cast<const f4 *>(Ar + (half * R + r) * K4 + k);
#pragma unroll
            for (int e = 0; e < 4; ++e) l1[r] += fabsf(av[e] - bv[e]);
        }
    }
#pragma unroll
    for (int r = 0; r < R; ++r) {
        const int rr = rb + half * R + r;
        const bool valid = jl < nj && half * R + r < nr;
        int b = ORDER_NB - 1;
        if (l1[r] > 0.f) {
            const float v = 4.f * (1.f - log2f(l1[r]));
            b = v < 0.f ? 0 : (v > float(ORDER_NB - 2) ? ORDER_NB - 2 : int(v));
            if (collapse) b = 0;
        } else if (row_begin + rr * row_step != jb + jl) {
            b = ORDER_NB - 2;
        }
        if (valid) bucket[(size_t)rr * N + jb + jl] = (unsigned char)b;
        (void)lds_count_aggregated(lh, b, valid);
    }
    __syncthreads();
    for (int i = threadIdx.x; i < ORDER_NB; i += blockDim.x) if (lh[i]) atomicAdd(&hist[i], lh[i]);
}

constexpr int PREP_SETUP_BLOCKS = 64;
template <class C>
__global__ void __launch_bounds__(256) sinkhorn_prep_kernel(const double *__restrict__ Msrc, int K, int RT, double reg,
                                                            typename C::T *__restrict__ img, const double *__restrict__ Psrc,
                                                            typename C::T *__restrict__ Pdst, int N, int write_tail, double stop_thr,
                                                            double floor_ulps, int n_tiles,
                                                            int n_rows, int row_begin, int row_step,
                                                            unsigned char *__restrict__ bucket, int *__restrict__ hist, int collapse) {
    extern __shared__ __attribute__((aligned(16))) unsigned char order_smem[];
    if ((int)blockIdx.x < n_tiles) {
        bucket_body(blockIdx.x, Psrc, N, K, n_rows, row_begin, row_step, bucket, hist, collapse, order_smem);
    } else {
        setup_body<C>(Msrc, K, RT, reg, img, Psrc, Pdst, (long)N * RT * C::TILE, write_tail, stop_thr, floor_ulps,
                      ((int)blockIdx.x - n_tiles) * (int)blockDim.x + (int)threadIdx.x, PREP_SETUP_BLOCKS * (int)blockDim.x,
                      hist - (CTRL_INTS - CTRL_UNEQUAL));
    }
}

static __global__ void order_scatter_kernel(const unsigned char *__restrict__ bucket, int n_items, const int *__restrict__ hist,
                                     int *__restrict__ cursor, int *__restrict__ list, int *__restrict__ split,
                                     int *__restrict__ main_queue_head, int solo_mode) {
    __shared__ int offs[ORDER_NB], lh[ORDER_NB], lbase[ORDER_NB], gh[ORDER_NB];
    if (threadIdx.x < ORDER_NB) { lh[threadIdx.x] = 0; gh[threadIdx.x] = hist[threadIdx.x]; }
    __syncthreads();
    if (threadIdx.x < ORDER_NB) {
        int run = 0;
        for (int b = ORDER_NB - 1; b > (int)threadIdx.x; --b) run += gh[b];
        offs[threadIdx.x] = run;
    }
    if (blockIdx.x == 0 && threadIdx.x == 64) {
        const int n_dup = (solo_mode & 2) ? gh[ORDER_NB - 1] : 0;
        split[0] = n_dup; split[1] = n_dup; split[2] = n_dup; split[3] = n_dup;
        *main_queue_head = n_dup;
    }
    __syncthreads();
    const int chunk = (n_items + gridDim.x - 1) / gridDim.x;
    const int q0 = blockIdx.x * chunk, q1 = (q0 + chunk < n_items) ? q0 + chunk : n_items;
    const int n_it = (q1 - q0 + (int)blockDim.x - 1) / (int)blockDim.x;
    for (int it = 0; it < n_it; ++it) {
        const int q = q0 + it * blockDim.x + threadIdx.x;
        const bool valid = q < q1;
        (void)lds_count_aggregated(lh, valid ? bucket[q] : 0, valid);
    }
    __syncthreads();
    if (threadIdx.x < ORDER_NB) {
        const int c = lh[threadIdx.x];
        lbase[threadIdx.x] = offs[threadIdx.x] + (c ? atomicAdd(&cursor[threadIdx.x], c) : 0);
        lh[threadIdx.x] = 0;
    }
    __syncthreads();
    for (int it = 0; it < n_it; ++it) {
        const int q = q0 + it * blockDim.x + threadIdx.x;
        const bool valid = q < q1;
        const int b = valid ? bucket[q] : 0;
        const int slot = lds_count_aggregated(lh, b, valid);
        if (valid) list[lbase[b] + slot] = q;
    }
}

}
```

### pilot_amd/csrc/sinkhorn_launch.hpp

```cpp
#pragma once
#include <hip/hip_runtime.h>
#include "sinkhorn_kernels.hpp"

namespace pilot {

enum { CFG_F32 = 0, CFG_F64 = 1, CFG_S32 = 2, CFG_H32 = 3 };

hipError_t launch_stream_f32(int RT, bool sym, bool track, dim3 grid, size_t lds, hipStream_t s, const GridParams &p);
hipError_t launch_stream_f64(int RT, bool sym, bool track, dim3 grid, size_t lds, hipStream_t s, const GridParams &p);
hipError_t launch_solo_track_f64(dim3 grid, hipStream_t s, const GridParams &p);
hipError_t launch_stream_s32(int RT, bool sym, bool track, int live1, dim3 grid, size_t lds, hipStream_t s, const GridParams &p);
hipError_t launch_stream_h32(int RT, bool sym, int live1, dim3 grid, size_t lds, hipStream_t s, const GridParams &p);
hipError_t launch_stream_tv(int cfg, int tv, int RT, bool sym, bool track, dim3 grid, size_t lds, hipStream_t s, const GridParams &p);
hipError_t launch_prep(int cfg, const double *M, int K, int RT, double reg, void *img, const double *P, void *Pslot, int N, int write_tail,
                       double stop_thr, double floor_ulps, int n_rows, int row_begin, int row_step, unsigned char *bucket, int *hist, int *list, int *split,
                       int *main_queue_head, int mode, int n_blocks, hipStream_t s);
hipError_t launch_wide(dim3 grid, hipStream_t s, const GridParams &p, float *rec);
hipError_t launch_wide_value(dim3 grid, hipStream_t s, const GridParams &p, const float *rec);
size_t wide_rec_elems();
hipError_t launch_quad(dim3 grid, hipStream_t s, const GridParams &p);
bool quad_covers(int K, bool sym);
size_t img_elems(int cfg, int RT);
size_t form_elems_rt(int cfg, int RT);
size_t track_img_elems(int cfg, int RT);

}
```

### pilot_amd/csrc/sk_inst.hip

```cpp
#include "sinkhorn_launch.hpp"

namespace pilot {
namespace {

template <class C, int RT, bool SYM, bool TRACK, int TV = 0>
hipError_t stream_one(dim3 grid, size_t lds, hipStream_t s, const GridParams &p) {
    auto kern = sinkhorn_stream_kernel<C, RT, SYM, TRACK, TV>;
    if (lds > 32 * 1024) {
        hipError_t e = hipFuncSetAttribute(reinterpret_cast<const void *>(kern), hipFuncAttributeMaxDynamicSharedMemorySize, (int)lds);
        if (e != hipSuccess) return e;
    }
    hipLaunchKernelGGL(kern, grid, dim3(WAVE * WAVES_PER_WG), lds, s, p);
    return hipGetLastError();
}
template <class C, int RT, int TV = 0>
hipError_t stream_rt(bool sym, bool track, dim3 grid, size_t lds, hipStream_t s, const GridParams &p) {
    if (track) return sym ? stream_one<C, RT, true, true, TV>(grid, lds, s, p) : stream_one<C, RT, false, true, TV>(grid, lds, s, p);
    return sym ? stream_one<C, RT, true, false, TV>(grid, lds, s, p) : stream_one<C, RT, false, false, TV>(grid, lds, s, p);
}
template <class C, int TV = 0>
hipError_t stream_any(int RT, bool sym, bool track, dim3 grid, size_t lds, hipStream_t s, const GridParams &p) {
    switch (RT) {
    case 1: if constexpr (TV == 0) return stream_rt<C, 1, TV>(sym, track, grid, lds, s, p); else return hipErrorInvalidValue;
    case 2: return stream_rt<C, 2, TV>(sym, track, grid, lds, s, p);
    case 3: return stream_rt<C, 3, TV>(sym, track, grid, lds, s, p);
    case 4: return stream_rt<C, 4, TV>(sym, track, grid, lds, s, p);
    case 5: return stream_rt<C, 5, TV>(sym, track, grid, lds, s, p);
    case 6: return stream_rt<C, 6, TV>(sym, track, grid, lds, s, p);
    case 7: return stream_rt<C, 7, TV>(sym, track, grid, lds, s, p);
    case 8: return stream_rt<C, 8, TV>(sym, track, grid, lds, s, p);
    default: return hipErrorInvalidValue;
    }
}

template <class C>
hipError_t prep_any(const double *M, int K, int RT, double reg, void *img, const double *P, void *Pslot, int N, int write_tail,
                    double stop_thr, double floor_ulps, int n_rows, int row_begin, int row_step, unsigned char *bucket, int *hist, int *list, int *split,
                    int *main_queue_head, int mode, int n_blocks, hipStream_t s) {
    using T = typename C::T;
    const int collapse = (mode >> 2) & 1;
    const int tiles = n_rows > 0 ? ((N + ORDER_JW - 1) / ORDER_JW) * ((n_rows + ORDER_RI - 1) / ORDER_RI) : 0;
    const int K4 = (K + 3) & ~3;
    const size_t lds = sizeof(float) * ((size_t)K4 * (ORDER_JW + 1) + (size_t)ORDER_RI * K4) + sizeof(int) * ORDER_NB;
    static bool attr_set[64] = {};
    int dev = 0;
    if (hipGetDevice(&dev) != hipSuccess || dev < 0 || dev >= 64) dev = 0;
    if (!attr_set[dev]) {
        hipError_t e = hipFuncSetAttribute(reinterpret_cast<const void *>(sinkhorn_prep_kernel<C>),
                                           hipFuncAttributeMaxDynamicSharedMemorySize, 150 * 1024);
        if (e != hipSuccess) return e;
        attr_set[dev] = true;
    }
    hipLaunchKernelGGL(sinkhorn_prep_kernel<C>, dim3(tiles + PREP_SETUP_BLOCKS), dim3(256), lds, s, M, K, RT, reg, static_cast<T *>(img), P,
                       static_cast<T *>(Pslot), N, write_tail, stop_thr, floor_ulps, tiles, n_rows, row_begin, row_step, bucket, hist, collapse);
    if (n_rows > 0)
        hipLaunchKernelGGL(order_scatter_kernel, dim3(n_blocks), dim3(256), 0, s, bucket, n_rows * N, hist, hist + ORDER_NB, list, split,
                           main_queue_head, mode & 3);
    return hipGetLastError();
}
}

#if SK_PART == 0
hipError_t launch_stream_f32(int RT, bool sym, bool track, dim3 grid, size_t lds, hipStream_t s, const GridParams &p) {
    return stream_any<CfgF32x16>(RT, sym, track, grid, lds, s, p);
}
hipError_t launch_prep_f64(const double *M, int K, int RT, double reg, void *img, const double *P, void *Pslot, int N, int write_tail,
                           double stop_thr, double floor_ulps, int n_rows, int row_begin, int row_step, unsigned char *bucket, int *hist, int *list, int *split,
                           int *main_queue_head, int mode, int n_blocks, hipStream_t s);
hipError_t launch_prep_s32(const double *M, int K, int RT, double reg, void *img, const double *P, void *Pslot, int N, int write_tail,
                           double stop_thr, double floor_ulps, int n_rows, int row_begin, int row_step, unsigned char *bucket, int *hist, int *list, int *split,
                           int *main_queue_head, int mode, int n_blocks, hipStream_t s);
hipError_t launch_prep_h32(const double *M, int K, int RT, double reg, void *img, const double *P, void *Pslot, int N, int write_tail,
                           double stop_thr, double floor_ulps, int n_rows, int row_begin, int row_step, unsigned char *bucket, int *hist, int *list, int *split,
                           int *main_queue_head, int mode, int n_blocks, hipStream_t s);
hipError_t launch_prep(int cfg, const double *M, int K, int RT, double reg, void *img, const double *P, void *Pslot, int N, int write_tail,
                       double stop_thr, double floor_ulps, int n_rows, int row_begin, int row_step, unsigned char *bucket, int *hist, int *list, int *split,
                       int *main_queue_head, int mode, int n_blocks, hipStream_t s) {
    if (cfg == CFG_F64)
        return launch_prep_f64(M, K, RT, reg, img, P, Pslot, N, write_tail, stop_thr, floor_ulps, n_rows, row_begin, row_step, bucket, hist, list, split,
                               main_queue_head, mode, n_blocks, s);
    if (cfg == CFG_H32)
        return launch_prep_h32(M, K, RT, reg, img, P, Pslot, N, write_tail, stop_thr, floor_ulps, n_rows, row_begin, row_step, bucket, hist, list, split,
                               main_queue_head, mode, n_blocks, s);
    if (cfg == CFG_S32)
        return launch_prep_s32(M, K, RT, reg, img, P, Pslot, N, write_tail, stop_thr, floor_ulps, n_rows, row_begin, row_step, bucket, hist, list, split,
                               main_queue_head, mode, n_blocks, s);
    return prep_any<CfgF32x16>(M, K, RT, reg, img, P, Pslot, N, write_tail, stop_thr, floor_ulps, n_rows, row_begin, row_step, bucket, hist, list, split,
                               main_queue_head, mode, n_blocks, s);
}
size_t form_elems_rt(int cfg, int RT) {
    if (cfg == CFG_H32) return (size_t)form_elems<CfgH32x16>(RT);
    return cfg == CFG_S32 ? (size_t)form_elems<CfgS32x16>(RT) : (cfg == CFG_F64 ? (size_t)form_elems<CfgF64x16>(RT) : (size_t)form_elems<CfgF32x16>(RT));
}
size_t track_img_elems(int cfg, int RT) { return cfg == CFG_H32 ? (size_t)track_img_offset<CfgH32x16>(RT) : 0; }
size_t img_elems(int cfg, int RT) {
    if (cfg == CFG_H32) return (size_t)img_total<CfgH32x16>(RT);
    return cfg == CFG_S32 ? (size_t)img_total<CfgS32x16>(RT) : (cfg == CFG_F64 ? (size_t)img_total<CfgF64x16>(RT) : (size_t)img_total<CfgF32x16>(RT));
}
#define PILOT_TV_DECL(NAME) \
    hipError_t launch_stream_##NAME(int RT, bool sym, bool track, dim3 grid, size_t lds, hipStream_t s, const GridParams &p);
PILOT_TV_DECL(f32_tv1) PILOT_TV_DECL(f32_tv2) PILOT_TV_DECL(f64_tv1) PILOT_TV_DECL(f64_tv2)
#undef PILOT_TV_DECL
hipError_t launch_stream_tv(int cfg, int tv, int RT, bool sym, bool track, dim3 grid, size_t lds, hipStream_t s, const GridParams &p) {
    if (cfg == CFG_F32) return tv == 1 ? launch_stream_f32_tv1(RT, sym, track, grid, lds, s, p) : launch_stream_f32_tv2(RT, sym, track, grid, lds, s, p);
    return tv == 1 ? launch_stream_f64_tv1(RT, sym, track, grid, lds, s, p) : launch_stream_f64_tv2(RT, sym, track, grid, lds, s, p);
}
#elif SK_PART == 1
hipError_t launch_stream_f64(int RT, bool sym, bool track, dim3 grid, size_t lds, hipStream_t s, const GridParams &p) {
    return stream_any<CfgF64x16>(RT, sym, track, grid, lds, s, p);
}
hipError_t launch_solo_track_f64(dim3 grid, hipStream_t s, const GridParams &p) {
    hipLaunchKernelGGL(sinkhorn_solo_track_kernel<CfgF64x16>, grid, dim3(WAVE * WAVES_PER_WG), sizeof(double) * WAVE * WAVES_PER_WG, s, p);
    return hipGetLastError();
}
hipError_t launch_prep_f64(const double *M, int K, int RT, double reg, void *img, const double *P, void *Pslot, int N, int write_tail,
                           double stop_thr, double floor_ulps, int n_rows, int row_begin, int row_step, unsigned char *bucket, int *hist, int *list, int *split,
                           int *main_queue_head, int mode, int n_blocks, hipStream_t s) {
    return prep_any<CfgF64x16>(M, K, RT, reg, img, P, Pslot, N, write_tail, stop_thr, floor_ulps, n_rows, row_begin, row_step, bucket, hist, list, split,
                               main_queue_head, mode, n_blocks, s);
}
#elif SK_PART == 7
hipError_t launch_stream_s32_l1(int RT, bool sym, bool track, dim3 grid, size_t lds, hipStream_t s, const GridParams &p) {
    return stream_any<CfgS32x16, 1>(RT, sym, track, grid, lds, s, p);
}
#elif SK_PART == 9
hipError_t launch_stream_h32_l1(int RT, bool sym, dim3 grid, size_t lds, hipStream_t s, const GridParams &p) {
    switch (RT) {
    case 2: return sym ? stream_one<CfgH32x16, 2, true, false, 1>(grid, lds, s, p) : stream_one<CfgH32x16, 2, false, false, 1>(grid, lds, s, p);
    case 3: return sym ? stream_one<CfgH32x16, 3, true, false, 1>(grid, lds, s, p) : stream_one<CfgH32x16, 3, false, false, 1>(grid, lds, s, p);
    case 4: return sym ? stream_one<CfgH32x16, 4, true, false, 1>(grid, lds, s, p) : stream_one<CfgH32x16, 4, false, false, 1>(grid, lds, s, p);
    default: return hipErrorInvalidValue;
    }
}
#elif SK_PART == 8
hipError_t launch_stream_h32_l1(int RT, bool sym, dim3 grid, size_t lds, hipStream_t s, const GridParams &p);
hipError_t launch_stream_h32(int RT, bool sym, int live1, dim3 grid, size_t lds, hipStream_t s, const GridParams &p) {
    if (live1) return launch_stream_h32_l1(RT, sym, grid, lds, s, p);
    switch (RT) {
    case 1: return sym ? stream_one<CfgH32x16, 1, true, false>(grid, lds, s, p) : stream_one<CfgH32x16, 1, false, false>(grid, lds, s, p);
    case 2: return sym ? stream_one<CfgH32x16, 2, true, false>(grid, lds, s, p) : stream_one<CfgH32x16, 2, false, false>(grid, lds, s, p);
    case 3: return sym ? stream_one<CfgH32x16, 3, true, false>(grid, lds, s, p) : stream_one<CfgH32x16, 3, false, false>(grid, lds, s, p);
    case 4: return sym ? stream_one<CfgH32x16, 4, true, false>(grid, lds, s, p) : stream_one<CfgH32x16, 4, false, false>(grid, lds, s, p);
    case 5: return sym ? stream_one<CfgH32x16, 5, true, false>(grid, lds, s, p) : stream_one<CfgH32x16, 5, false, false>(grid, lds, s, p);
    case 6: return sym ? stream_one<CfgH32x16, 6, true, false>(grid, lds, s, p) : stream_one<CfgH32x16, 6, false, false>(grid, lds, s, p);
    case 7: return sym ? stream_one<CfgH32x16, 7, true, false>(grid, lds, s, p) : stream_one<CfgH32x16, 7, false, false>(grid, lds, s, p);
    case 8: return sym ? stream_one<CfgH32x16, 8, true, false>(grid, lds, s, p) : stream_one<CfgH32x16, 8, false, false>(grid, lds, s, p);
    default: return hipErrorInvalidValue;
    }
}
hipError_t launch_prep_h32(const double *M, int K, int RT, double reg, void *img, const double *P, void *Pslot, int N, int write_tail,
                           double stop_thr, double floor_ulps, int n_rows, int row_begin, int row_step, unsigned char *bucket, int *hist, int *list, int *split,
                           int *main_queue_head, int mode, int n_blocks, hipStream_t s) {
    return prep_any<CfgH32x16>(M, K, RT, reg, img, P, Pslot, N, write_tail, stop_thr, floor_ulps, n_rows, row_begin, row_step, bucket, hist, list, split,
                               main_queue_head, mode, n_blocks, s);
}
#elif SK_PART == 6
hipError_t launch_stream_s32_l1(int RT, bool sym, bool track, dim3 grid, size_t lds, hipStream_t s, const GridParams &p);
hipError_t launch_stream_s32(int RT, bool sym, bool track, int live1, dim3 grid, size_t lds, hipStream_t s, const GridParams &p) {
    if (live1) return launch_stream_s32_l1(RT, sym, track, grid, lds, s, p);
    return stream_any<CfgS32x16>(RT, sym, track, grid, lds, s, p);
}
hipError_t launch_prep_s32(const double *M, int K, int RT, double reg, void *img, const double *P, void *Pslot, int N, int write_tail,
                           double stop_thr, double floor_ulps, int n_rows, int row_begin, int row_step, unsigned char *bucket, int *hist, int *list, int *split,
                           int *main_queue_head, int mode, int n_blocks, hipStream_t s) {
    return prep_any<CfgS32x16>(M, K, RT, reg, img, P, Pslot, N, write_tail, stop_thr, floor_ulps, n_rows, row_begin, row_step, bucket, hist, list, split,
                               main_queue_head, mode, n_blocks, s);
}
#else
#if SK_PART == 2
#define PILOT_TV_CFG CfgF32x16
#define PILOT_TV_N 1
#define PILOT_TV_NAME(x) x##f32_tv1
#elif SK_PART == 3
#define PILOT_TV_CFG CfgF32x16
#define PILOT_TV_N 2
#define PILOT_TV_NAME(x) x##f32_tv2
#elif SK_PART == 4
#define PILOT_TV_CFG CfgF64x16
#define PILOT_TV_N 1
#define PILOT_TV_NAME(x) x##f64_tv1
#else
#define PILOT_TV_CFG CfgF64x16
#define PILOT_TV_N 2
#define PILOT_TV_NAME(x) x##f64_tv2
#endif
hipError_t PILOT_TV_NAME(launch_stream_)(int RT, bool sym, bool track, dim3 grid, size_t lds, hipStream_t s, const GridParams &p) {
    return stream_any<PILOT_TV_CFG, PILOT_TV_N>(RT, sym, track, grid, lds, s, p);
}
#endif

}
```

Before: 548.8 million.

## Fuse bucket rank computation into prep and simplify order scatter, batch prep loads

The bucketing pass now records each pair's within-bucket position by reserving global histogram ranges per tile, so the scatter kernel becomes a single-pass, one-thread-per-item write instead of a two-pass per-block count and atomic cursor scheme. Prep loops batch global loads into register arrays to expose more memory-level parallelism, and the setup block count is raised. The per-call memset of control counters is moved off the hot path: counters are zeroed once at allocation and reset at the end of runs (by the last generic block or on fallback paths). This adds a pos buffer (reusing track_list) and relies on the counters being left clean across calls.

Result: faster. 559.9 million, median of 6 (+2.0%).

```diff
diff --git a/pilot_amd/csrc/generic_kernels.hpp b/pilot_amd/csrc/generic_kernels.hpp
--- a/pilot_amd/csrc/generic_kernels.hpp
+++ b/pilot_amd/csrc/generic_kernels.hpp
@@ -17,6 +17,8 @@
     const int *list;
     const int *list_len;
     int nsplit;
+    int *ctrl;
+    int ctrl_ints;
 };
 
 #ifndef PILOT_GENERIC_WG
@@ -76,12 +78,14 @@
         __threadfence_block();
         __syncthreads();
     };
+    const int n_items = PLAN ? 0 : (p.list_len ? *p.list_len : p.n_pairs);
+    int last_draw = 0;
     for (;;) {
         if (threadIdx.x == 0) qs[0] = atomicAdd(p.queue, 1);
         __syncthreads();
         const int item = qs[0];
         __syncthreads();
-        if (item >= (PLAN ? pa->n_pairs : (p.list_len ? *p.list_len : p.n_pairs))) break;
+        if (item >= (PLAN ? pa->n_pairs : n_items)) { last_draw = item; break; }
         const int q = PLAN ? item : p.list ? p.list[item] : item;
         const int i_s = PLAN ? pa->pair_i[item] : p.row_begin + (q / N) * p.row_step, j_s = PLAN ? pa->pair_j[item] : q % N;
         for (int k = threadIdx.x; k < K; k += GENERIC_WG) {
@@ -186,6 +190,10 @@
         }
         __syncthreads();
     }
+    if constexpr (!PLAN) {
+        if (p.ctrl && last_draw == n_items + (int)gridDim.x - 1)
+            for (int i = threadIdx.x; i < p.ctrl_ints; i += GENERIC_WG) __hip_atomic_store(p.ctrl + i, 0, __ATOMIC_RELAXED, __HIP_MEMORY_SCOPE_AGENT);
+    }
 }
 
 }
diff --git a/pilot_amd/csrc/pilot_ot.hip b/pilot_amd/csrc/pilot_ot.hip
--- a/pilot_amd/csrc/pilot_ot.hip
+++ b/pilot_amd/csrc/pilot_ot.hip
@@ -456,6 +456,8 @@
     }
     if (e == hipSuccess) e = hipMalloc(reinterpret_cast<void **>(&pl->track_list), sizeof(int) * (size_t)N * N);
     if (e == hipSuccess) e = hipMalloc(reinterpret_cast<void **>(&pl->track_count), CTRL_BLOCK_INTS * sizeof(int));
+    if (e == hipSuccess) e = hipMemset(pl->track_count, 0, CTRL_BLOCK_INTS * sizeof(int));
+    if (e == hipSuccess) e = hipStreamSynchronize(nullptr);
     if (e == hipSuccess) e = hipMalloc(reinterpret_cast<void **>(&pl->order_list), sizeof(int) * (size_t)N * N);
     if (e == hipSuccess) e = hipMalloc(reinterpret_cast<void **>(&pl->order_bucket), (size_t)N * N);
     if (e == hipSuccess) e = hipMalloc(reinterpret_cast<void **>(&pl->emd_counter), sizeof(int) * pilot::EMD_NQ * pilot::EMD_Q_STRIDE);
@@ -553,6 +555,7 @@
     g.reg = reg; g.tau = tau; g.stop_thr = stop_thr; g.max_iter = num_iter_max; g.period = check_period;
     g.emd = d_emd; g.iters = d_iters; g.err = d_err; g.flags = d_flags; g.kws = pl->kws; g.queue = queue; g.nsplit = nsplit;
     g.list = list; g.list_len = list_len;
+    g.ctrl = pl->track_count; g.ctrl_ints = CTRL_BLOCK_INTS;
     int wgs = pl->generic_wgs < n_pairs ? pl->generic_wgs : n_pairs;
     if (list && wgs > 64) wgs = 64;
     if (const char *e = pilot::test_switch("PILOT_OT_GENERIC_WGS")) { const int w = atoi(e); if (w > 0 && w < wgs) wgs = w; }
@@ -631,7 +634,6 @@
         return fail(PILOT_OT_ENOTSUP, "K=%d with a %ssymmetric cost needs %zu B of LDS (> %zu) in this precision", K, sym ? "" : "non-",
                     fixed + pilot::WAVES_PER_WG * slot_bytes, LDS_BYTES);
     pl->order_hist = pl->track_count + CTRL_INTS;
-    HIP_TRY(hipMemsetAsync(pl->track_count, 0, CTRL_BLOCK_INTS * sizeof(int), s));
     void *img = pl->img;
     void *Pt = pl->p_slot;
     if (n_rows == 0) return PILOT_OT_OK;
@@ -679,12 +681,10 @@
     const bool solo = stream_has_solo(w, RT, sym, tv, split, half) && !(p.debug & 512) && !track_all && full_tiles < 3 * wave_slots;
     int solo_blocks = 0;
     {
-        int ob = (n_pairs + 1023) / 1024;
-        if (ob > pl->n_cu) ob = pl->n_cu;
         int *split_ctl = pl->track_count + 4;
         const int mode = (solo ? 2 : 0) | ((p.debug & 2) ? 4 : 0);
         HIP_TRY(pilot::launch_prep(cfg, d_M, K, RT, reg, img, d_P, Pt, N, (tv ? 1 : 0) | 2 | (mixed ? 4 : 0), stop_thr, floor_ulps, n_rows, row_begin, row_step,
-                                   pl->order_bucket, pl->order_hist, pl->order_list, split_ctl, pl->track_count + 1, mode, ob, s));
+                                   pl->order_bucket, pl->track_list, pl->order_hist, pl->order_list, split_ctl, pl->track_count + 1, mode, s));
         p.list = pl->order_list;
         if (solo) {
             solo_blocks = (n_rows + pilot::WAVES_PER_WG - 1) / pilot::WAVES_PER_WG;
@@ -756,7 +756,7 @@
         if (fixed64 + pilot::WAVES_PER_WG * slot64 > LDS_BYTES)
             return fail(PILOT_OT_ENOTSUP, "K=%d: the f64 fallback needs %zu B of LDS", K, fixed64 + pilot::WAVES_PER_WG * slot64);
         HIP_TRY(pilot::launch_prep(pilot::CFG_F64, d_M, K, RT64, reg, img, d_P, Pt, N, 2, stop_thr, floor_ulps, 0, row_begin, row_step,
-                                   pl->order_bucket, pl->order_hist, pl->order_list, pl->track_count + 4, pl->track_count + 1, 0, 1, s));
+                                   pl->order_bucket, nullptr, pl->order_hist, pl->order_list, pl->track_count + 4, pl->track_count + 1, 0, s));
         pilot::GridParams q = p;
         q.list = mixed ? pl->track_list : fb_list; q.list_len = pl->track_count + 8; q.queue_head = pl->track_count + 9; q.queue_shards = nullptr;
         q.img = img;
@@ -778,6 +778,8 @@
         const int rc = run_generic(pl, d_P, d_M, reg, num_iter_max, stop_thr, tau, check_period, row_begin, n_rows, row_step, d_emd, d_iters,
                                    d_err, d_flags, s, pl->nan_list, pl->track_count + 10, pl->track_count + 11);
         if (rc != PILOT_OT_OK) return rc;
+    } else {
+        HIP_TRY(hipMemsetAsync(pl->track_count, 0, CTRL_BLOCK_INTS * sizeof(int), s));
     }
     return PILOT_OT_OK;
 }
@@ -824,10 +826,8 @@
         HIP_TRY(hipMalloc(reinterpret_cast<void **>(&pl->wide_rec), sizeof(float) * pilot::wide_rec_elems() * (size_t)n_pairs));
         pl->wide_rec_n = (size_t)n_pairs;
     }
-    int ob = (n_pairs + 1023) / 1024;
-    if (ob > pl->n_cu) ob = pl->n_cu;
     HIP_TRY(pilot::launch_prep(pilot::CFG_H32, d_M, K, RT, reg, pl->img, d_P, pl->p_slot, N, 0, stop_thr, floor_ulps, n_rows, row_begin, row_step,
-                               pl->order_bucket, pl->order_hist, pl->order_list, pl->track_count + 4, pl->track_count + 1, 0, ob, s));
+                               pl->order_bucket, pl->track_list, pl->order_hist, pl->order_list, pl->track_count + 4, pl->track_count + 1, 0, s));
     pilot::GridParams p;
     p.P = pl->p_slot; p.img = pl->img; p.N = N; p.K = K;
     p.n_pairs = n_pairs;
@@ -896,6 +896,7 @@
     auto run = [&](hipStream_t on) {
         int r = run_grid(cfg, pl, d_P, d_M, reg, num_iter_max, stop_thr, tau, check_period, f32_floor_ulps, cost_is_symmetric != 0,
                          row_begin, n_rows, row_step, d_emd, d_iters, d_err, d_flags, on, mixed);
+        if (r != PILOT_OT_OK) (void)hipMemsetAsync(pl->track_count, 0, CTRL_BLOCK_INTS * sizeof(int), on);
         if (r == PILOT_OT_ENOTSUP)
             r = run_generic(pl, d_P, d_M, reg, num_iter_max, stop_thr, tau, check_period, row_begin, n_rows, row_step, d_emd, d_iters, d_err,
                             d_flags, on);
diff --git a/pilot_amd/csrc/sinkhorn_kernels.hpp b/pilot_amd/csrc/sinkhorn_kernels.hpp
--- a/pilot_amd/csrc/sinkhorn_kernels.hpp
+++ b/pilot_amd/csrc/sinkhorn_kernels.hpp
@@ -1577,6 +1577,8 @@
         }
     }
 }
+constexpr int PREP_BATCH = 16, PREP_ROW_BATCH = 32;
+
 template <class C>
 __device__ inline void write_first_product(const double *__restrict__ Msrc, int K, int RT, double reg, typename C::T *__restrict__ tab,
                                            double scale, int tid, int nthr) {
@@ -1591,7 +1593,13 @@
         const int j = M::lidx(t, r, g);
         double s = 0.0;
         if (j < K)
-            for (int k = part; k < K; k += 4) s += exp(-Msrc[(size_t)k * K + j] / reg);
+            for (int k0 = part; k0 < K; k0 += 4 * PREP_BATCH) {
+                double m[PREP_BATCH];
+#pragma unroll
+                for (int u = 0; u < PREP_BATCH; ++u) { const int k = k0 + 4 * u < K ? k0 + 4 * u : K - 1; m[u] = Msrc[(size_t)k * K + j]; }
+#pragma unroll
+                for (int u = 0; u < PREP_BATCH; ++u) if (k0 + 4 * u < K) s += exp(-m[u] / reg);
+            }
         s += __shfl_xor(s, 1);
         s += __shfl_xor(s, 2);
         if (part == 0) tab[slot] = T(j < K ? s / K * scale : 1.0);
@@ -1665,10 +1673,24 @@
         }
     }
     double mass0 = 0.0;
-    for (int k = 0; k < K; ++k) mass0 += Psrc[k];
+    if (tid < n_p / KP) {
+        for (int k0 = 0; k0 < K; k0 += PREP_ROW_BATCH) {
+            double x[PREP_ROW_BATCH];
+#pragma unroll
+            for (int u = 0; u < PREP_ROW_BATCH; ++u) x[u] = Psrc[k0 + u < K ? k0 + u : K - 1];
+#pragma unroll
+            for (int u = 0; u < PREP_ROW_BATCH; ++u) if (k0 + u < K) mass0 += x[u];
+        }
+    }
     for (long row = tid; row < n_p / KP; row += nthr) {
         double n2 = 0.0, mass = 0.0;
-        for (int k = 0; k < K; ++k) { n2 += Psrc[row * K + k] * Psrc[row * K + k]; mass += Psrc[row * K + k]; }
+        for (int k0 = 0; k0 < K; k0 += PREP_ROW_BATCH) {
+            double x[PREP_ROW_BATCH];
+#pragma unroll
+            for (int u = 0; u < PREP_ROW_BATCH; ++u) x[u] = Psrc[row * K + (k0 + u < K ? k0 + u : K - 1)];
+#pragma unroll
+            for (int u = 0; u < PREP_ROW_BATCH; ++u) if (k0 + u < K) { n2 += x[u] * x[u]; mass += x[u]; }
+        }
         if (unequal && !(fabs(mass - mass0) <= 1e-6 * fabs(mass0))) atomicOr(unequal, 1);
         double thr = stop_thr;
         if (sizeof(T) == 4) { const double fl = floor_ulps * 1.1920928955078125e-07 * sqrt(n2); thr = thr > fl ? thr : fl; }
@@ -1708,20 +1730,27 @@
 constexpr int ORDER_JW = 128, ORDER_RI = 8;
 
 __device__ inline void bucket_body(int tile, const double *__restrict__ Psrc, int N, int K, int n_rows, int row_begin,
-                                   int row_step, unsigned char *__restrict__ bucket, int *__restrict__ hist, int collapse,
-                                   unsigned char *order_smem) {
+                                   int row_step, unsigned char *__restrict__ bucket, int *__restrict__ pos, int *__restrict__ hist,
+                                   int collapse, unsigned char *order_smem) {
     const int K4 = (K + 3) & ~3;
     float *Bt = reinterpret_cast<float *>(order_smem);
     float *Ar = Bt + (size_t)K4 * (ORDER_JW + 1);
     int *lh = reinterpret_cast<int *>(Ar + ORDER_RI * K4);
+    int *lbase = lh + ORDER_NB;
     const int n_jb = (N + ORDER_JW - 1) / ORDER_JW;
     const int jb = (tile % n_jb) * ORDER_JW, rb = (tile / n_jb) * ORDER_RI;
     const int nj = N - jb < ORDER_JW ? N - jb : ORDER_JW;
     const int nr = n_rows - rb < ORDER_RI ? n_rows - rb : ORDER_RI;
     for (int e = threadIdx.x; e < ORDER_NB; e += blockDim.x) lh[e] = 0;
-    for (int e = threadIdx.x; e < nj * K; e += blockDim.x) {
-        const int row = e / K, k = e % K;
-        Bt[k * (ORDER_JW + 1) + row] = float(Psrc[(size_t)jb * K + e]);
+    for (int e0 = threadIdx.x; e0 < nj * K; e0 += PREP_BATCH * blockDim.x) {
+        double x[PREP_BATCH];
+#pragma unroll
+        for (int u = 0; u < PREP_BATCH; ++u) { const int e = e0 + u * (int)blockDim.x; x[u] = Psrc[(size_t)jb * K + (e < nj * K ? e : nj * K - 1)]; }
+#pragma unroll
+        for (int u = 0; u < PREP_BATCH; ++u) {
+            const int e = e0 + u * (int)blockDim.x;
+            if (e < nj * K) Bt[(e % K) * (ORDER_JW + 1) + e / K] = float(x[u]);
+        }
     }
     for (int e = threadIdx.x; e < (K4 - K) * ORDER_JW; e += blockDim.x) Bt[(K + e / ORDER_JW) * (ORDER_JW + 1) + e % ORDER_JW] = 0.f;
     for (int e = threadIdx.x; e < ORDER_RI * K4; e += blockDim.x) {
@@ -1746,6 +1775,7 @@
             for (int e = 0; e < 4; ++e) l1[r] += fabsf(av[e] - bv[e]);
         }
     }
+    int bk[R], rank[R];
 #pragma unroll
     for (int r = 0; r < R; ++r) {
         const int rr = rb + half * R + r;
@@ -1759,23 +1789,31 @@
             b = ORDER_NB - 2;
         }
         if (valid) bucket[(size_t)rr * N + jb + jl] = (unsigned char)b;
-        (void)lds_count_aggregated(lh, b, valid);
+        bk[r] = b;
+        rank[r] = lds_count_aggregated(lh, b, valid);
     }
     __syncthreads();
-    for (int i = threadIdx.x; i < ORDER_NB; i += blockDim.x) if (lh[i]) atomicAdd(&hist[i], lh[i]);
-}
-
-constexpr int PREP_SETUP_BLOCKS = 64;
+    for (int i = threadIdx.x; i < ORDER_NB; i += blockDim.x) lbase[i] = lh[i] ? atomicAdd(&hist[i], lh[i]) : 0;
+    __syncthreads();
+#pragma unroll
+    for (int r = 0; r < R; ++r) {
+        const int rr = rb + half * R + r;
+        if (jl < nj && half * R + r < nr) pos[(size_t)rr * N + jb + jl] = lbase[bk[r]] + rank[r];
+    }
+}
+
+constexpr int PREP_SETUP_BLOCKS = 160;
 template <class C>
 __global__ void __launch_bounds__(256) sinkhorn_prep_kernel(const double *__restrict__ Msrc, int K, int RT, double reg,
                                                             typename C::T *__restrict__ img, const double *__restrict__ Psrc,
                                                             typename C::T *__restrict__ Pdst, int N, int write_tail, double stop_thr,
                                                             double floor_ulps, int n_tiles,
                                                             int n_rows, int row_begin, int row_step,
-                                                            unsigned char *__restrict__ bucket, int *__restrict__ hist, int collapse) {
+                                                            unsigned char *__restrict__ bucket, int *__restrict__ pos,
+                                                            int *__restrict__ hist, int collapse) {
     extern __shared__ __attribute__((aligned(16))) unsigned char order_smem[];
     if ((int)blockIdx.x < n_tiles) {
-        bucket_body(blockIdx.x, Psrc, N, K, n_rows, row_begin, row_step, bucket, hist, collapse, order_smem);
+        bucket_body(blockIdx.x, Psrc, N, K, n_rows, row_begin, row_step, bucket, pos, hist, collapse, order_smem);
     } else {
         setup_body<C>(Msrc, K, RT, reg, img, Psrc, Pdst, (long)N * RT * C::TILE, write_tail, stop_thr, floor_ulps,
                       ((int)blockIdx.x - n_tiles) * (int)blockDim.x + (int)threadIdx.x, PREP_SETUP_BLOCKS * (int)blockDim.x,
@@ -1783,15 +1821,19 @@
     }
 }
 
-static __global__ void order_scatter_kernel(const unsigned char *__restrict__ bucket, int n_items, const int *__restrict__ hist,
-                                     int *__restrict__ cursor, int *__restrict__ list, int *__restrict__ split,
-                                     int *__restrict__ main_queue_head, int solo_mode) {
-    __shared__ int offs[ORDER_NB], lh[ORDER_NB], lbase[ORDER_NB], gh[ORDER_NB];
-    if (threadIdx.x < ORDER_NB) { lh[threadIdx.x] = 0; gh[threadIdx.x] = hist[threadIdx.x]; }
+static __global__ void __launch_bounds__(256) order_scatter_kernel(const unsigned char *__restrict__ bucket, const int *__restrict__ pos,
+                                                                   int n_items, const int *__restrict__ hist, int *__restrict__ list,
+                                                                   int *__restrict__ split, int *__restrict__ main_queue_head, int solo_mode) {
+    __shared__ int offs[ORDER_NB], gh[ORDER_NB];
+    const long qq = (long)blockIdx.x * blockDim.x + threadIdx.x;
+    const bool valid = qq < n_items;
+    const int q = (int)qq;
+    const int b = valid ? bucket[q] : 0, at = valid ? pos[q] : 0;
+    if (threadIdx.x < ORDER_NB) gh[threadIdx.x] = hist[threadIdx.x];
     __syncthreads();
     if (threadIdx.x < ORDER_NB) {
         int run = 0;
-        for (int b = ORDER_NB - 1; b > (int)threadIdx.x; --b) run += gh[b];
+        for (int c = ORDER_NB - 1; c > (int)threadIdx.x; --c) run += gh[c];
         offs[threadIdx.x] = run;
     }
     if (blockIdx.x == 0 && threadIdx.x == 64) {
@@ -1800,28 +1842,7 @@
         *main_queue_head = n_dup;
     }
     __syncthreads();
-    const int chunk = (n_items + gridDim.x - 1) / gridDim.x;
-    const int q0 = blockIdx.x * chunk, q1 = (q0 + chunk < n_items) ? q0 + chunk : n_items;
-    const int n_it = (q1 - q0 + (int)blockDim.x - 1) / (int)blockDim.x;
-    for (int it = 0; it < n_it; ++it) {
-        const int q = q0 + it * blockDim.x + threadIdx.x;
-        const bool valid = q < q1;
-        (void)lds_count_aggregated(lh, valid ? bucket[q] : 0, valid);
-    }
-    __syncthreads();
-    if (threadIdx.x < ORDER_NB) {
-        const int c = lh[threadIdx.x];
-        lbase[threadIdx.x] = offs[threadIdx.x] + (c ? atomicAdd(&cursor[threadIdx.x], c) : 0);
-        lh[threadIdx.x] = 0;
-    }
-    __syncthreads();
-    for (int it = 0; it < n_it; ++it) {
-        const int q = q0 + it * blockDim.x + threadIdx.x;
-        const bool valid = q < q1;
-        const int b = valid ? bucket[q] : 0;
-        const int slot = lds_count_aggregated(lh, b, valid);
-        if (valid) list[lbase[b] + slot] = q;
-    }
-}
-
-}
+    if (valid) list[offs[b] + at] = q;
+}
+
+}
diff --git a/pilot_amd/csrc/sinkhorn_launch.hpp b/pilot_amd/csrc/sinkhorn_launch.hpp
--- a/pilot_amd/csrc/sinkhorn_launch.hpp
+++ b/pilot_amd/csrc/sinkhorn_launch.hpp
@@ -13,8 +13,8 @@
 hipError_t launch_stream_h32(int RT, bool sym, int live1, dim3 grid, size_t lds, hipStream_t s, const GridParams &p);
 hipError_t launch_stream_tv(int cfg, int tv, int RT, bool sym, bool track, dim3 grid, size_t lds, hipStream_t s, const GridParams &p);
 hipError_t launch_prep(int cfg, const double *M, int K, int RT, double reg, void *img, const double *P, void *Pslot, int N, int write_tail,
-                       double stop_thr, double floor_ulps, int n_rows, int row_begin, int row_step, unsigned char *bucket, int *hist, int *list, int *split,
-                       int *main_queue_head, int mode, int n_blocks, hipStream_t s);
+                       double stop_thr, double floor_ulps, int n_rows, int row_begin, int row_step, unsigned char *bucket, int *pos, int *hist, int *list, int *split,
+                       int *main_queue_head, int mode, hipStream_t s);
 hipError_t launch_wide(dim3 grid, hipStream_t s, const GridParams &p, float *rec);
 hipError_t launch_wide_value(dim3 grid, hipStream_t s, const GridParams &p, const float *rec);
 size_t wide_rec_elems();
diff --git a/pilot_amd/csrc/sk_inst.hip b/pilot_amd/csrc/sk_inst.hip
--- a/pilot_amd/csrc/sk_inst.hip
+++ b/pilot_amd/csrc/sk_inst.hip
@@ -35,13 +35,13 @@
 
 template <class C>
 hipError_t prep_any(const double *M, int K, int RT, double reg, void *img, const double *P, void *Pslot, int N, int write_tail,
-                    double stop_thr, double floor_ulps, int n_rows, int row_begin, int row_step, unsigned char *bucket, int *hist, int *list, int *split,
-                    int *main_queue_head, int mode, int n_blocks, hipStream_t s) {
+                    double stop_thr, double floor_ulps, int n_rows, int row_begin, int row_step, unsigned char *bucket, int *pos, int *hist, int *list, int *split,
+                    int *main_queue_head, int mode, hipStream_t s) {
     using T = typename C::T;
     const int collapse = (mode >> 2) & 1;
     const int tiles = n_rows > 0 ? ((N + ORDER_JW - 1) / ORDER_JW) * ((n_rows + ORDER_RI - 1) / ORDER_RI) : 0;
     const int K4 = (K + 3) & ~3;
-    const size_t lds = sizeof(float) * ((size_t)K4 * (ORDER_JW + 1) + (size_t)ORDER_RI * K4) + sizeof(int) * ORDER_NB;
+    const size_t lds = sizeof(float) * ((size_t)K4 * (ORDER_JW + 1) + (size_t)ORDER_RI * K4) + sizeof(int) * 2 * ORDER_NB;
     static bool attr_set[64] = {};
     int dev = 0;
     if (hipGetDevice(&dev) != hipSuccess || dev < 0 || dev >= 64) dev = 0;
@@ -52,10 +52,12 @@
         attr_set[dev] = true;
     }
     hipLaunchKernelGGL(sinkhorn_prep_kernel<C>, dim3(tiles + PREP_SETUP_BLOCKS), dim3(256), lds, s, M, K, RT, reg, static_cast<T *>(img), P,
-                       static_cast<T *>(Pslot), N, write_tail, stop_thr, floor_ulps, tiles, n_rows, row_begin, row_step, bucket, hist, collapse);
-    if (n_rows > 0)
-        hipLaunchKernelGGL(order_scatter_kernel, dim3(n_blocks), dim3(256), 0, s, bucket, n_rows * N, hist, hist + ORDER_NB, list, split,
-                           main_queue_head, mode & 3);
+                       static_cast<T *>(Pslot), N, write_tail, stop_thr, floor_ulps, tiles, n_rows, row_begin, row_step, bucket, pos, hist, collapse);
+    if (n_rows > 0) {
+        const int n_items = n_rows * N;
+        hipLaunchKernelGGL(order_scatter_kernel, dim3((unsigned)((n_items + 255) / 256)), dim3(256), 0, s, bucket, pos, n_items, hist, list,
+                           split, main_queue_head, mode & 3);
+    }
     return hipGetLastError();
 }
 }
@@ -65,28 +67,28 @@
     return stream_any<CfgF32x16>(RT, sym, track, grid, lds, s, p);
 }
 hipError_t launch_prep_f64(const double *M, int K, int RT, double reg, void *img, const double *P, void *Pslot, int N, int write_tail,
-                           double stop_thr, double floor_ulps, int n_rows, int row_begin, int row_step, unsigned char *bucket, int *hist, int *list, int *split,
-                           int *main_queue_head, int mode, int n_blocks, hipStream_t s);
+                           double stop_thr, double floor_ulps, int n_rows, int row_begin, int row_step, unsigned char *bucket, int *pos, int *hist, int *list, int *split,
+                           int *main_queue_head, int mode, hipStream_t s);
 hipError_t launch_prep_s32(const double *M, int K, int RT, double reg, void *img, const double *P, void *Pslot, int N, int write_tail,
-                           double stop_thr, double floor_ulps, int n_rows, int row_begin, int row_step, unsigned char *bucket, int *hist, int *list, int *split,
-                           int *main_queue_head, int mode, int n_blocks, hipStream_t s);
+                           double stop_thr, double floor_ulps, int n_rows, int row_begin, int row_step, unsigned char *bucket, int *pos, int *hist, int *list, int *split,
+                           int *main_queue_head, int mode, hipStream_t s);
 hipError_t launch_prep_h32(const double *M, int K, int RT, double reg, void *img, const double *P, void *Pslot, int N, int write_tail,
-                           double stop_thr, double floor_ulps, int n_rows, int row_begin, int row_step, unsigned char *bucket, int *hist, int *list, int *split,
-                           int *main_queue_head, int mode, int n_blocks, hipStream_t s);
+                           double stop_thr, double floor_ulps, int n_rows, int row_begin, int row_step, unsigned char *bucket, int *pos, int *hist, int *list, int *split,
+                           int *main_queue_head, int mode, hipStream_t s);
 hipError_t launch_prep(int cfg, const double *M, int K, int RT, double reg, void *img, const double *P, void *Pslot, int N, int write_tail,
-                       double stop_thr, double floor_ulps, int n_rows, int row_begin, int row_step, unsigned char *bucket, int *hist, int *list, int *split,
-                       int *main_queue_head, int mode, int n_blocks, hipStream_t s) {
+                       double stop_thr, double floor_ulps, int n_rows, int row_begin, int row_step, unsigned char *bucket, int *pos, int *hist, int *list, int *split,
+                       int *main_queue_head, int mode, hipStream_t s) {
     if (cfg == CFG_F64)
-        return launch_prep_f64(M, K, RT, reg, img, P, Pslot, N, write_tail, stop_thr, floor_ulps, n_rows, row_begin, row_step, bucket, hist, list, split,
-                               main_queue_head, mode, n_blocks, s);
+        return launch_prep_f64(M, K, RT, reg, img, P, Pslot, N, write_tail, stop_thr, floor_ulps, n_rows, row_begin, row_step, bucket, pos, hist, list, split,
+                               main_queue_head, mode, s);
     if (cfg == CFG_H32)
-        return launch_prep_h32(M, K, RT, reg, img, P, Pslot, N, write_tail, stop_thr, floor_ulps, n_rows, row_begin, row_step, bucket, hist, list, split,
-                               main_queue_head, mode, n_blocks, s);
+        return launch_prep_h32(M, K, RT, reg, img, P, Pslot, N, write_tail, stop_thr, floor_ulps, n_rows, row_begin, row_step, bucket, pos, hist, list, split,
+                               main_queue_head, mode, s);
     if (cfg == CFG_S32)
-        return launch_prep_s32(M, K, RT, reg, img, P, Pslot, N, write_tail, stop_thr, floor_ulps, n_rows, row_begin, row_step, bucket, hist, list, split,
-                               main_queue_head, mode, n_blocks, s);
-    return prep_any<CfgF32x16>(M, K, RT, reg, img, P, Pslot, N, write_tail, stop_thr, floor_ulps, n_rows, row_begin, row_step, bucket, hist, list, split,
-                               main_queue_head, mode, n_blocks, s);
+        return launch_prep_s32(M, K, RT, reg, img, P, Pslot, N, write_tail, stop_thr, floor_ulps, n_rows, row_begin, row_step, bucket, pos, hist, list, split,
+                               main_queue_head, mode, s);
+    return prep_any<CfgF32x16>(M, K, RT, reg, img, P, Pslot, N, write_tail, stop_thr, floor_ulps, n_rows, row_begin, row_step, bucket, pos, hist, list, split,
+                               main_queue_head, mode, s);
 }
 size_t form_elems_rt(int cfg, int RT) {
     if (cfg == CFG_H32) return (size_t)form_elems<CfgH32x16>(RT);
@@ -114,10 +116,10 @@
     return hipGetLastError();
 }
 hipError_t launch_prep_f64(const double *M, int K, int RT, double reg, void *img, const double *P, void *Pslot, int N, int write_tail,
-                           double stop_thr, double floor_ulps, int n_rows, int row_begin, int row_step, unsigned char *bucket, int *hist, int *list, int *split,
-                           int *main_queue_head, int mode, int n_blocks, hipStream_t s) {
-    return prep_any<CfgF64x16>(M, K, RT, reg, img, P, Pslot, N, write_tail, stop_thr, floor_ulps, n_rows, row_begin, row_step, bucket, hist, list, split,
-                               main_queue_head, mode, n_blocks, s);
+                           double stop_thr, double floor_ulps, int n_rows, int row_begin, int row_step, unsigned char *bucket, int *pos, int *hist, int *list, int *split,
+                           int *main_queue_head, int mode, hipStream_t s) {
+    return prep_any<CfgF64x16>(M, K, RT, reg, img, P, Pslot, N, write_tail, stop_thr, floor_ulps, n_rows, row_begin, row_step, bucket, pos, hist, list, split,
+                               main_queue_head, mode, s);
 }
 #elif SK_PART == 7
 hipError_t launch_stream_s32_l1(int RT, bool sym, bool track, dim3 grid, size_t lds, hipStream_t s, const GridParams &p) {
@@ -149,10 +151,10 @@
     }
 }
 hipError_t launch_prep_h32(const double *M, int K, int RT, double reg, void *img, const double *P, void *Pslot, int N, int write_tail,
-                           double stop_thr, double floor_ulps, int n_rows, int row_begin, int row_step, unsigned char *bucket, int *hist, int *list, int *split,
-                           int *main_queue_head, int mode, int n_blocks, hipStream_t s) {
-    return prep_any<CfgH32x16>(M, K, RT, reg, img, P, Pslot, N, write_tail, stop_thr, floor_ulps, n_rows, row_begin, row_step, bucket, hist, list, split,
-                               main_queue_head, mode, n_blocks, s);
+                           double stop_thr, double floor_ulps, int n_rows, int row_begin, int row_step, unsigned char *bucket, int *pos, int *hist, int *list, int *split,
+                           int *main_queue_head, int mode, hipStream_t s) {
+    return prep_any<CfgH32x16>(M, K, RT, reg, img, P, Pslot, N, write_tail, stop_thr, floor_ulps, n_rows, row_begin, row_step, bucket, pos, hist, list, split,
+                               main_queue_head, mode, s);
 }
 #elif SK_PART == 6
 hipError_t launch_stream_s32_l1(int RT, bool sym, bool track, dim3 grid, size_t lds, hipStream_t s, const GridParams &p);
@@ -161,10 +163,10 @@
     return stream_any<CfgS32x16>(RT, sym, track, grid, lds, s, p);
 }
 hipError_t launch_prep_s32(const double *M, int K, int RT, double reg, void *img, const double *P, void *Pslot, int N, int write_tail,
-                           double stop_thr, double floor_ulps, int n_rows, int row_begin, int row_step, unsigned char *bucket, int *hist, int *list, int *split,
-                           int *main_queue_head, int mode, int n_blocks, hipStream_t s) {
-    return prep_any<CfgS32x16>(M, K, RT, reg, img, P, Pslot, N, write_tail, stop_thr, floor_ulps, n_rows, row_begin, row_step, bucket, hist, list, split,
-                               main_queue_head, mode, n_blocks, s);
+                           double stop_thr, double floor_ulps, int n_rows, int row_begin, int row_step, unsigned char *bucket, int *pos, int *hist, int *list, int *split,
+                           int *main_queue_head, int mode, hipStream_t s) {
+    return prep_any<CfgS32x16>(M, K, RT, reg, img, P, Pslot, N, write_tail, stop_thr, floor_ulps, n_rows, row_begin, row_step, bucket, pos, hist, list, split,
+                               main_queue_head, mode, s);
 }
 #else
 #if SK_PART == 2
```
